# HuiGuanLab/Lite-MKD

Hardware: AMD Instinct MI355X
Metric: episodes/sec (5-way 5-shot, 8x224^2 frames) (higher is better)
Workload: dtype f32

## Files before the change

lite-mkd_amd/csrc/conv.hip:

```cpp
#include "gemm_core.h"
#include <atomic>
#include <mutex>

struct ConvGemmArgs {
  const float* src;
  const float* wpk;
  float* out;
  float* stat_partial;
  int N, Hs, Ws, Cs;
  int Hr, Wr, rows_per_class, tiles_per_class;
  int sh;
  int Ho, Wo, Co, omul;
  int Kp, cps, nclass;
  int n_rt, n_ct, xcd_mode;
  int taps_pm1;
  int grid_step;
  int grid_total;
  int same;
  int halo;
  int accum;
  const float* ep_stats;
  const float* ep_res;
  int ep_relu;
  const float* pre_stats;
// ... 130 lines not shown
    }
    if (ok) {
      s_src[r] = ((n * a.Hs + aa * a.sh) * a.Ws + bb * a.sh) * a.Cs;
      s_hw[r] = ((aa * a.sh) << 16) | (bb * a.sh);
      s_out[r] = ((n * a.Ho + aa * a.omul + ph) * a.Wo + bb * a.omul + pw) * a.Co;
    } else {
      s_src[r] = 0;
      s_hw[r] = -1;
      s_out[r] = -1;
    }
  }
  __syncthreads();
  LA la;
  LB lb;
  la.init(a.src, a.Hs, a.Ws, a.Cs, s_src, s_hw);
  lb.init(a.wpk, a.Kp, n0, a.Co, a.Kp);

  f32x16 acc[Cfg::TM][Cfg::TN];
  const int nk = a.ntap[cls] * a.cps;
  {
    constexpr int SA = LA::LDS_FLOATS, SB = LB::LDS_FLOATS;
    float* As0 = smem;
    float* Bs0 = smem + 2 * SA;
    const int lane = tid & 63, wave = tid >> 6;
    const int wm = wave / Cfg::WN, wn = wave % Cfg::WN;
    const int h = lane >> 5;
    const int a_row = wm * (Cfg::TM * 32) + (lane & 31);
    const int b_row = wn * (Cfg::TN * 32) + (lane & 31);
#pragma unroll
    for (int i = 0; i < Cfg::TM; ++i)
#pragma unroll
      for (int j = 0; j < Cfg::TN; ++j)
#pragma unroll
        for (int e = 0; e < 16; ++e) acc[i][j][e] = 0.f;
    const Tap* taps = a.taps[cls];
    const int ntap_c = a.ntap[cls];
    auto issue = [&](int t) {
      const int cc = t / ntap_c, tp = t - cc * ntap_c;
      const Tap tap = taps[tp];
      if (PRE && tp == 0) la.load_pre(a.pre_stats, cc * LMKD_BK);
      la.load(tap.dh, tap.dw, cc * LMKD_BK);
      lb.load(tap.kofs + cc * LMKD_BK);
    };
    if (nk > 0) {
      issue(0);
      la.store(As0);
      lb.store(Bs0);
      __syncthreads();
      for (int t = 0; t + 1 < nk; ++t) {
        const int cur = t & 1;
        issue(t + 1);
        if (BF16) mfma_kstep_bf16<Cfg, LA, LB>(As0 + cur * SA, Bs0 + cur * SB, a_row, b_row, h, acc);
        else mfma_kstep<Cfg, LA, LB>(As0 + cur * SA, Bs0 + cur * SB, a_row, b_row, h, acc);
        __builtin_amdgcn_sched_barrier(0);
        la.store(As0 + (cur ^ 1) * SA);
        lb.store(Bs0 + (cur ^ 1) * SB);
        __syncthreads();
      }
      const int last = (nk - 1) & 1;
      if (BF16) mfma_kstep_bf16<Cfg, LA, LB>(As0 + last * SA, Bs0 + last * SB, a_row, b_row, h, acc);
      else mfma_kstep<Cfg, LA, LB>(As0 + last * SA, Bs0 + last * SB, a_row, b_row, h, acc);
    }
  }

  const int lane = tid & 63, wave = tid >> 6;
  const int wm = wave / Cfg::WN, wn = wave % Cfg::WN;
  const int cl0 = wn * (Cfg::TN * 32) + (lane & 31);
  if (STATS == 0 && a.accum) {
    float prev[Cfg::TM][Cfg::TN][16];
#pragma unroll
    for (int i = 0; i < Cfg::TM; ++i)
#pragma unroll
      for (int e = 0; e < 16; ++e) {
        const int ob = s_out[wm * (Cfg::TM * 32) + i * 32 + acc_row(e, lane)];
#pragma unroll
        for (int j = 0; j < Cfg::TN; ++j) {
          const int col = n0 + cl0 + j * 32;
          prev[i][j][e] = (ob >= 0 && col < a.Co) ? a.out[(long)ob + col] : 0.f;
        }
      }
#pragma unroll
    for (int i = 0; i < Cfg::TM; ++i)
#pragma unroll
      for (int j = 0; j < Cfg::TN; ++j)
#pragma unroll
        for (int e = 0; e < 16; ++e) acc[i][j][e] = acc[i][j][e] + prev[i][j][e];
  }
  float s1[Cfg::TN], s2[Cfg::TN];
#pragma unroll
  for (int j = 0; j < Cfg::TN; ++j) s1[j] = s2[j] = 0.f;
  float esc[Cfg::TN], esh[Cfg::TN];
  if (STATS == 2) {
#pragma unroll
    for (int j = 0; j < Cfg::TN; ++j) {
      const int col = n0 + cl0 + j * 32;
      esc[j] = col < a.Co ? a.ep_stats[2 * a.Co + col] : 0.f;
      esh[j] = col < a.Co ? a.ep_stats[3 * a.Co + col] : 0.f;
    }
  }
#pragma unroll
  for (int i = 0; i < Cfg::TM; ++i) {
#pragma unroll
    for (int e = 0; e < 16; ++e) {
      const int rl = wm * (Cfg::TM * 32) + i * 32 + acc_row(e, lane);
      const int ob = s_out[rl];
#pragma unroll
      for (int j = 0; j < Cfg::TN; ++j) {
        const int col = n0 + cl0 + j * 32;
        float v = acc[i][j][e];
        if (ob >= 0 && col < a.Co) {
          float* o = a.out + (long)ob + col;
          if (STATS == 2) {
            v = fmaf(v, esc[j], esh[j]);
            if (a.ep_res) v += a.ep_res[(long)ob + col];
            if (a.ep_relu) v = fmaxf(v, 0.f);
            *o = v;
          } else {
            *o = (STATS == 1 && a.accum) ? v + *o : v;
          }
        }
        if (STATS == 1) { s1[j] += v; s2[j] = fmaf(v, v, s2[j]); }
      }
    }
    __builtin_amdgcn_sched_barrier(0);
  }
  if (STATS == 1) {
#pragma unroll
    for (int j = 0; j < Cfg::TN; ++j) {
      const float t1 = s1[j] + __shfl_xor(s1[j], 32, 64);
      const float t2 = s2[j] + __shfl_xor(s2[j], 32, 64);
      if (lane < 32) {
        s_red[(wm * Cfg::BN + cl0 + j * 32) * 2 + 0] = t1;
        s_red[(wm * Cfg::BN + cl0 + j * 32) * 2 + 1] = t2;
      }
    }
  }
  if (STATS == 1) {
    __syncthreads();
    if (tid < Cfg::BN && n0 + tid < a.Co) {
      float s1 = 0.f, s2 = 0.f;
#pragma unroll
      for (int w = 0; w < Cfg::WM; ++w) {
        s1 += s_red[(w * Cfg::BN + tid) * 2 + 0];
        s2 += s_red[(w * Cfg::BN + tid) * 2 + 1];
      }
      float* p = a.stat_partial + ((long)rt * a.Co + n0 + tid) * 2;
      p[0] = s1;
      p[1] = s2;
    }
  }
}

#include "conv_x3.h"
#include "h2.h"
#include "conv_patch.h"
#include "conv_patch16.h"
#include "conv_stem.h"

struct WgradArgs {
  const float* dy;
  const float* x;
  float* slab;
  int N, Hs, Ws, Cs, Ho, Wo, Co;
  int stride, pad, KH, KW, KWp;
  int Kp, Mpix, steps_total, steps_per_split;
  int n_mt, n_jt, splits, xcd_mode;
  const float* pre_stats;
  int seg_pix0, seg_splits0, sps1;
  FastDiv div_hw, div_w;
  const unsigned* h2_xw;
  const unsigned* h2_dyw;
};

struct WinSlab { int kfirst, kend, nk, seg; };
__device__ __forceinline__ WinSlab win_slab(int z, int Mpix, int sps0, int seg_pix0, int seg_splits0, int sps1) {
  WinSlab w;
  int sps;
  if (z < seg_splits0) { w.kfirst = z * sps0 * LMKD_BK; w.kend = seg_pix0; w.seg = 0; sps = sps0; }
  else { w.kfirst = seg_pix0 + (z - seg_splits0) * sps1 * LMKD_BK; w.kend = Mpix; w.seg = 1; sps = sps1; }
  const int left = (w.kend - w.kfirst + LMKD_BK - 1) / LMKD_BK;
  w.nk = left < sps ? (left < 0 ? 0 : left) : sps;
  return w;
}

template <int ROWS, bool SMALLC, int THREADS = LMKD_THREADS, bool PRE = false>
struct LoaderWgradGather {
  static constexpr bool ROWK = false;
  static constexpr int LD = ROWS;
  static constexpr int LDS_FLOATS = LMKD_BK * LD;
  static constexpr int CPR = ROWS / 4;
  static constexpr int KPP = THREADS / CPR;
  static constexpr int NI = LMKD_BK / KPP;
  const float* x;
  FastDiv div_hw, div_w;
  int Mpix, HoWo, Wo, Hs, Ws, Cs, stride;
  float4 reg[NI];
  int dh, dw, coff, r4;
  bool tap_ok;
  float4 psc, psh;
  unsigned inb;
  __device__ __forceinline__ void init(const WgradArgs& a, int j0) {
    inb = 0u;
    x = a.x; div_hw = a.div_hw; div_w = a.div_w;
    Mpix = a.Mpix; HoWo = a.Ho * a.Wo; Wo = a.Wo; Hs = a.Hs; Ws = a.Ws; Cs = a.Cs; stride = a.stride;
    const int tid = threadIdx.x;
    r4 = (tid % CPR) * 4;
    const int col = j0 + r4;
    if (SMALLC) {
      const int kh = col >> 5, kw = (col & 31) >> 2;
      dh = kh - a.pad; dw = kw - a.pad; coff = 0;
      tap_ok = kh < a.KH && kw < a.KW && col < a.Kp;
    } else {
      const int tap = col / a.Cs;
      coff = col - tap * a.Cs;
      const int kh = tap / a.KWp, kw = tap - kh * a.KWp;
      dh = kh - a.pad; dw = kw - a.pad;
      tap_ok = col < a.Kp && kw < a.KW;
    }
    if (PRE && tap_ok) {
      psc = *reinterpret_cast<const float4*>(a.pre_stats + 2 * a.Cs + coff);
      psh = *reinterpret_cast<const float4*>(a.pre_stats + 3 * a.Cs + coff);
    }
  }
  __device__ __forceinline__ void load(int koff) {
    const int tid = threadIdx.x;
#pragma unroll
    for (int i = 0; i < NI; ++i) {
      const int p = koff + tid / CPR + KPP * i;
      float4 v = make_float4(0.f, 0.f, 0.f, 0.f);
      if (tap_ok && p < Mpix) {
        const int n = fdiv(p, div_hw);
        const int rem = p - n * HoWo;
        const int oh = fdiv(rem, div_w);
        const int ow = rem - oh * Wo;
        const int h = oh * stride + dh, w = ow * stride + dw;
        if ((unsigned)h < (unsigned)Hs && (unsigned)w < (unsigned)Ws) {
          v = *reinterpret_cast<const float4*>(x + ((long)(n * Hs + h) * Ws + w) * Cs + coff);
          if (PRE) inb |= 1u << i;
        } else if (PRE) inb &= ~(1u << i);
      } else if (PRE) inb &= ~(1u << i);
      reg[i] = v;
    }
  }
  __device__ __forceinline__ void store(float* S) const {
    const int tid = threadIdx.x;
#pragma unroll
    for (int i = 0; i < NI; ++i) {
      int k = tid / CPR + KPP * i;
      float4 v = reg[i];
      if (PRE && ((inb >> i) & 1u)) {
        v.x = fmaxf(fmaf(v.x, psc.x, psh.x), 0.f); v.y = fmaxf(fmaf(v.y, psc.y, psh.y), 0.f);
        v.z = fmaxf(fmaf(v.z, psc.z, psh.z), 0.f); v.w = fmaxf(fmaf(v.w, psc.w, psh.w), 0.f);
      }
      *reinterpret_cast<float4*>(S + k * LD + r4) = v;
    }
  }
};

template <class Cfg, bool SMALLC, bool BF16, bool PRE = false>
__global__ __launch_bounds__(Cfg::THREADS) void conv_wgrad_kernel(WgradArgs a) {
  using LA = LoaderMMajorDense<Cfg::BM, Cfg::THREADS>;
  using LB = LoaderWgradGather<Cfg::BN, SMALLC, Cfg::THREADS, PRE>;
  __shared__ __attribute__((aligned(16))) float smem[2 * (LA::LDS_FLOATS + LB::LDS_FLOATS)];
  int z, tz;
  const int tiles_per_z = a.n_mt * a.n_jt;
  if (a.xcd_mode) {
    const int xj = blockIdx.x >> 3;
    z = (blockIdx.x & 7) + 8 * (xj / tiles_per_z);
    if (z >= a.splits) return;
    tz = xj - (xj / tiles_per_z) * tiles_per_z;
  } else {
    z = blockIdx.x / tiles_per_z;
    tz = blockIdx.x - z * tiles_per_z;
  }
  const int m0 = (tz % a.n_mt) * Cfg::BM, j0 = (tz / a.n_mt) * Cfg::BN;
  LA la;
  LB lb;
  la.init(a.dy, a.Co, m0, a.Co, a.Mpix);
  lb.init(a, j0);
  const int s0 = z * a.steps_per_split;
  int nk = a.steps_total - s0;
  if (nk > a.steps_per_split) nk = a.steps_per_split;
  f32x16 acc[Cfg::TM][Cfg::TN];
  auto koff = [s0](int t) { return (s0 + t) * LMKD_BK; };
  gemm_mainloop<Cfg, LA, LB, decltype(koff), decltype(koff), BF16, PRE>(la, lb, nk, koff, koff, smem, acc);

  const int lane = threadIdx.x & 63, wave = threadIdx.x >> 6;
  const int wm = wave / Cfg::WN, wn = wave % Cfg::WN;
  float* C = a.slab + (long)z * a.Co * a.Kp;
#pragma unroll
  for (int j = 0; j < Cfg::TN; ++j) {
    const int col = j0 + wn * (Cfg::TN * 32) + j * 32 + (lane & 31);
    if (col >= a.Kp) continue;
#pragma unroll
    for (int i = 0; i < Cfg::TM; ++i)
#pragma unroll
      for (int e = 0; e < 16; ++e) {
        const int row = m0 + wm * (Cfg::TM * 32) + i * 32 + acc_row(e, lane);
        if (row < a.Co) C[(long)row * a.Kp + col] = acc[i][j][e];
      }
  }
}

__global__ void wgrad_reduce_kernel(const float* __restrict__ slab, float* __restrict__ dw, int splits, int Co, int Cin,
                                    int Cs, int KH, int KW, int KWp, int Kp, int accumulate) {
  const long total = (long)Co * KH * KW * Cin;
  const long zs = (long)Co * Kp;
  for (long idx = (long)blockIdx.x * blockDim.x + threadIdx.x; idx < total; idx += (long)gridDim.x * blockDim.x) {
    const int ci = idx % Cin;
    long r = idx / Cin;
    const int kw = r % KW; r /= KW;
    const int kh = r % KH;
    const int co = r / KH;
    const float* p = slab + (long)co * Kp + (long)(kh * KWp + kw) * Cs + ci;
    float s0 = 0.f, s1 = 0.f, s2 = 0.f, s3 = 0.f;
    int z = 0;
    for (; z + 8 <= splits; z += 8) {
      const float a0 = p[(z + 0) * zs], a1 = p[(z + 1) * zs], a2 = p[(z + 2) * zs], a3 = p[(z + 3) * zs];
      const float a4 = p[(z + 4) * zs], a5 = p[(z + 5) * zs], a6 = p[(z + 6) * zs], a7 = p[(z + 7) * zs];
      s0 += a0; s1 += a1; s2 += a2; s3 += a3; s0 += a4; s1 += a5; s2 += a6; s3 += a7;
    }
    for (; z < splits; ++z) s0 += p[z * zs];
    float* o = dw + (((long)co * Cin + ci) * KH + kh) * KW + kw;
    const float v = (s0 + s1) + (s2 + s3);
    *o = accumulate ? *o + v : v;
  }
}

__global__ __launch_bounds__(1024) void wgrad_reduce_stem_kernel(const float* __restrict__ slab, float* __restrict__ dw, int splits, int Co, int Cin,
                                                                 int Cs, int KH, int KW, int KWp, int Kp, int accumulate) {
  __shared__ float sm[4][256];
  const int k = threadIdx.x, q = threadIdx.y, co = blockIdx.x;
  const long zs = (long)Co * Kp;
  float s0 = 0.f, s1 = 0.f, s2 = 0.f, s3 = 0.f;
  if (k < Kp) {
    const float* p = slab + (long)co * Kp + k;
    int z = q;
    for (; z + 28 < splits; z += 32) {
      const float a0 = p[(z + 0) * zs], a1 = p[(z + 4) * zs], a2 = p[(z + 8) * zs], a3 = p[(z + 12) * zs];
      const float a4 = p[(z + 16) * zs], a5 = p[(z + 20) * zs], a6 = p[(z + 24) * zs], a7 = p[(z + 28) * zs];
      s0 += a0; s1 += a1; s2 += a2; s3 += a3; s0 += a4; s1 += a5; s2 += a6; s3 += a7;
    }
    for (; z < splits; z += 4) s0 += p[z * zs];
  }
  sm[q][k] = (s0 + s1) + (s2 + s3);
  __syncthreads();
  if (q == 0 && k < Kp) {
    const int ci = k % Cs, r = k / Cs;
    const int kw = r % KWp, kh = r / KWp;
    if (ci < Cin && kw < KW && kh < KH) {
      const float v = (sm[0][k] + sm[1][k]) + (sm[2][k] + sm[3][k]);
      float* o = dw + (((long)co * Cin + ci) * KH + kh) * KW + kw;
      *o = accumulate ? *o + v : v;
    }
  }
}
static void launch_wgrad_reduce(const float* slab, float* dw, int splits, int Co, int Cin, int Cs, int KH, int KW, int KWp, int Kp,
                                int accumulate, hipStream_t s) {
  const long total = (long)Co * KH * KW * Cin;
  int rg = cdiv(total, 256);
  if (rg > 4096) rg = 4096;
  hipLaunchKernelGGL(wgrad_reduce_kernel, dim3(rg), dim3(256), 0, s, slab, dw, splits, Co, Cin, Cs, KH, KW, KWp, Kp, accumulate);
}

#include "wgrad_x3.h"
#include "wgrad_win.h"
#include "wgrad_stem.h"

__global__ void pack_weights_kernel(const float* __restrict__ w, float* __restrict__ wp, int Co, int Cin, int Cs, int KH,
                                    int KW, int KWp, int mode) {
  if (mode == 0) {
    const long total = (long)Co * KH * KWp * Cs;
    for (long idx = (long)blockIdx.x * blockDim.x + threadIdx.x; idx < total; idx += (long)gridDim.x * blockDim.x) {
      const int ci = idx % Cs;
      long r = idx / Cs;
      const int kw = r % KWp; r /= KWp;
      const int kh = r % KH;
      const int co = r / KH;
      wp[idx] = (ci < Cin && kw < KW) ? w[(((long)co * Cin + ci) * KH + kh) * KW + kw] : 0.f;
    }
  } else {
    const long total = (long)Cin * KH * KW * Co;
    for (long idx = (long)blockIdx.x * blockDim.x + threadIdx.x; idx < total; idx += (long)gridDim.x * blockDim.x) {
      const int co = idx % Co;
      long r = idx / Co;
      const int kw = r % KW; r /= KW;
      const int kh = r % KH;
      const int ci = r / KH;
      wp[idx] = w[(((long)co * Cin + ci) * KH + kh) * KW + kw];
    }
  }
}

static inline int conv_out(int H, int K, int s, int p) { return (H + 2 * p - K) / s + 1; }
static inline int kw_padded(int Cs, int KW) { return Cs >= 32 ? KW : ((KW * Cs + 31) / 32) * 32 / Cs; }

extern "C" long lmkd_conv2d_packed_weight_elems(int Cout, int Cin, int Cs, int KH, int KW, int mode) {
  if (mode == 0) return (long)Cout * KH * kw_padded(Cs, KW) * Cs;
  return (long)Cin * KH * KW * Cout;
}

extern "C" int lmkd_conv2d_pack_weights(const float* w_oihw, float* wp, int Cout, int Cin, int Cs, int KH, int KW,
                                        int mode, void* stream) {
  LMKD_REQUIRE(w_oihw && wp, "lmkd_conv2d_pack_weights: null pointer");
  LMKD_REQUIRE(mode == 0 || mode == 1, "lmkd_conv2d_pack_weights: mode must be 0 (fwd) or 1 (dgrad)");
  LMKD_REQUIRE(Cs >= Cin && (Cs % 32 == 0 || Cs == 4), "lmkd_conv2d_pack_weights: Cs=%d must be 4 or a multiple of 32", Cs);
  const long total = lmkd_conv2d_packed_weight_elems(Cout, Cin, Cs, KH, KW, mode);
  int grid = cdiv(total, 256);
  if (grid > 4096) grid = 4096;
  hipLaunchKernelGGL(pack_weights_kernel, dim3(grid), dim3(256), 0, (hipStream_t)stream, w_oihw, wp, Cout, Cin, Cs, KH, KW,
                     kw_padded(Cs, KW), mode);
  LMKD_CHECK_LAUNCH("lmkd_conv2d_pack_weights");
  return LMKD_OK;
}

static int g_conv_mode = 2;
static std::atomic<long> g_h2_launches{0};
static std::atomic<long> g_h2_fallbacks{0};
extern "C" long lmkd_conv_h2_launches(void) { return g_h2_launches.load(); }
extern "C" long lmkd_conv_h2_fallbacks(void) { return g_h2_fallbacks.load(); }
extern "C" int lmkd_conv_set_compute_dtype(int mode) {
  LMKD_REQUIRE(mode >= 0 && mode <= 4, "lmkd_conv_set_compute_dtype: 0 fp32 MFMA, 1 bf16, 2 fp32 as 3xbf16 (6 products), 3 (9 products), 4 fp32 as 2xfp16 (3 products) over mode 2");
  g_conv_mode = mode;
  return LMKD_OK;
}
extern "C" int lmkd_conv_get_compute_dtype(void) { return g_conv_mode; }
static inline int conv_nprod(bool act16 = false, bool maxima = false) {
  if (act16) return 1;
  switch (g_conv_mode) {
    case 0: return 0;
    case 1: return 1;
    case 3: return 9;
    case 4: return maxima ? 3 : 6;
    default: return 6;
  }
}
static inline bool conv_planes() { return conv_nprod() != 0; }
static inline bool conv_h2() { return conv_nprod(false, true) == 3; }
static inline void note_fenced(const lmkd_amax_desc* am) { if (conv_h2() && am && (am->flags & LMKD_AMAX_FENCED)) ++g_h2_fallbacks; }
extern "C" long lmkd_conv2d_plane_elems(int ncols, int Kp) {
  const long n = (long)ncols * Kp;
  return conv_nprod() == 1 ? n : (conv_h2() ? 18 * n + 32 : 12 * n);
}
static int amax_impl(const float* x, long n, void* word, int slots, void* stream, bool zero = true) {
  LMKD_REQUIRE(x && word && n > 0, "lmkd_amax: bad arguments");
  if (zero && hipMemsetAsync(word, 0, slots ? LMKD_AMAX_SEG_WORDS * 4 : 4, (hipStream_t)stream) != hipSuccess) {
    lmkd_set_error("lmkd_amax: hipMemsetAsync failed");
    return LMKD_EHIP;
  }
  int grid = cdiv(n, 256 * 16);
  if (grid > 2048) grid = 2048;
  if (slots) hipLaunchKernelGGL(amax_kernel<true>, dim3(grid), dim3(256), 0, (hipStream_t)stream, x, n, (unsigned*)word);
  else hipLaunchKernelGGL(amax_kernel<false>, dim3(grid), dim3(256), 0, (hipStream_t)stream, x, n, (unsigned*)word);
  LMKD_CHECK_LAUNCH("amax_kernel");
  return LMKD_OK;
}
extern "C" int lmkd_amax(const float* x, long n, void* word, void* stream) { return amax_impl(x, n, word, 1, stream); }

extern "C" int lmkd_conv2d_split_weights(const float* wp, void* wf, int ncols, int Kp, void* stream) {
  LMKD_REQUIRE(wp && wf, "lmkd_conv2d_split_weights: null pointer");
  LMKD_REQUIRE(ncols > 0 && ncols % 32 == 0 && Kp > 0 && Kp % 32 == 0, "lmkd_conv2d_split_weights: ncols=%d and Kp=%d must be multiples of 32", ncols, Kp);
  LMKD_REQUIRE((long)ncols * Kp * 24 < 0xffffffe0L, "lmkd_conv2d_split_weights: weights exceed the 4 GiB buffer range");
  int grid = cdiv((long)ncols * Kp, 256);
  if (grid > 4096) grid = 4096;
  hipLaunchKernelGGL(split_weights_kernel, dim3(grid), dim3(256), 0, (hipStream_t)stream, wp, (unsigned short*)wf, ncols, Kp,
                     conv_nprod() == 1 ? 1 : 3);
  LMKD_CHECK_LAUNCH("split_weights_kernel");
  if (conv_nprod() != 1) {
    hipLaunchKernelGGL(split_weights16_kernel, dim3(grid), dim3(256), 0, (hipStream_t)stream, wp, (unsigned short*)wf + (long)ncols * Kp * 6, ncols, Kp);
    LMKD_CHECK_LAUNCH("split_weights16_kernel");
  }
  if (conv_h2()) {
    unsigned short* wh = (unsigned short*)wf + (long)ncols * Kp * 12;
    const int rc = amax_impl(wp, (long)ncols * Kp, wh + (long)ncols * Kp * 4, 0, stream);
    if (rc) return rc;
    hipLaunchKernelGGL(split_weights16_h2_kernel, dim3(grid), dim3(256), 0, (hipStream_t)stream, wp, wh, ncols, Kp);
    LMKD_CHECK_LAUNCH("split_weights16_h2_kernel");
    hipLaunchKernelGGL(split_weights_h2_32_kernel, dim3(grid), dim3(256), 0, (hipStream_t)stream, wp, wh, ncols, Kp);
    LMKD_CHECK_LAUNCH("split_weights_h2_32_kernel");
  }
  return LMKD_OK;
}

struct RepackEntry {
  const float* w;
  unsigned short* wf;
  int Co, Cin, Cs, KH, KW, KWp, mode, ncols, Kp;
};
#define LMKD_REPACK_MAX 40
struct RepackArgs {
  RepackEntry e[LMKD_REPACK_MAX];
  int npl;
};
__device__ __forceinline__ float repack_fetch(const RepackEntry& e, int col, int k) {
  if (e.mode == 0) {
    const int ci = k % e.Cs;
    const int r = k / e.Cs;
    const int kw = r % e.KWp, kh = r / e.KWp;
    return (ci < e.Cin && kw < e.KW) ? e.w[(((long)col * e.Cin + ci) * e.KH + kh) * e.KW + kw] : 0.f;
  }
  const int co = k % e.Co;
  const int r = k / e.Co;
  const int kw = r % e.KW, kh = r / e.KW;
  return e.w[(((long)co * e.Cin + col) * e.KH + kh) * e.KW + kw];
}
__global__ void repack_h2_kernel(RepackArgs a, int phase) {
  const RepackEntry& e = a.e[blockIdx.y];
  const long total = (long)e.ncols * e.Kp;
  unsigned short* wh = e.wf + total * 12;
  unsigned* word = reinterpret_cast<unsigned*>(wh + total * 4);
  if (phase == 0) {
    if (blockIdx.x == 0 && threadIdx.x == 0) *word = 0u;
    return;
  }
  if (phase == 1) {
    float m = 0.f;
    for (long idx = (long)blockIdx.x * blockDim.x + threadIdx.x; idx < total; idx += (long)gridDim.x * blockDim.x) {
      const int col = (int)(idx / e.Kp), k = (int)(idx - (long)col * e.Kp);
      m = fmaxf(m, fabsf(repack_fetch(e, col, k)));
    }
#pragma unroll
    for (int o = 32; o >= 1; o >>= 1) m = fmaxf(m, __shfl_xor(m, o, 64));
    if ((threadIdx.x & 63) == 0) atomicMax(word, __float_as_uint(m));
    return;
  }
  const float s = h2_scale(*word);
  const int G16 = e.Kp >> 5, G = e.Kp >> 4;
  unsigned short* wh32 = wh + total * 4 + 32;
  for (long idx = (long)blockIdx.x * blockDim.x + threadIdx.x; idx < total; idx += (long)gridDim.x * blockDim.x) {
    const int col = (int)(idx / e.Kp), k = (int)(idx - (long)col * e.Kp);
    const int lane16 = (col & 15) + 16 * patch16_kslot((k >> 3) & 3);
    const long q = ((((long)(col >> 4) * G16 + (k >> 5)) * 2) * 64 + lane16) * 8 + (k & 7);
    unsigned short p0, p1;
    h2_split1(repack_fetch(e, col, k) * s, p0, p1);
    wh[q] = p0; wh[q + 512] = p1;
    const long q2 = q + total * 2;
    wh[q2] = p0 ^ 0x8000u; wh[q2 + 512] = p1 ^ 0x8000u;
    const long o = ((((long)(col >> 5) * G + (k >> 4)) * 2) * 64 + (col & 31) + 32 * ((k >> 3) & 1)) * 8 + (k & 7);
    wh32[o] = p0; wh32[o + 512] = p1;
  }
}
__global__ void repack_multi_kernel(RepackArgs a) {
  const RepackEntry& e = a.e[blockIdx.y];
  const long total = (long)e.ncols * e.Kp;
  const int G = e.Kp >> 4, G16 = e.Kp >> 5;
  for (long idx = (long)blockIdx.x * blockDim.x + threadIdx.x; idx < total; idx += (long)gridDim.x * blockDim.x) {
    const int col = (int)(idx / e.Kp), k = (int)(idx - (long)col * e.Kp);
    const float x = repack_fetch(e, col, k);
    const int lane = (col & 31) + 32 * ((k >> 3) & 1);
    const long o = ((((long)(col >> 5) * G + (k >> 4)) * a.npl) * 64 + lane) * 8 + (k & 7);
    if (a.npl == 1) {
      union { __bf16 h; unsigned short u; } c;
      c.h = (__bf16)x;
      e.wf[o] = c.u;
      continue;
    }
    const unsigned b0 = __float_as_uint(x);
    const float r1 = x - __uint_as_float(b0 & 0xffff0000u);
    const unsigned b1 = __float_as_uint(r1);
    const float r2 = r1 - __uint_as_float(b1 & 0xffff0000u);
    const unsigned short p0 = (unsigned short)(b0 >> 16), p1 = (unsigned short)(b1 >> 16), p2 = (unsigned short)(__float_as_uint(r2) >> 16);
    const unsigned short n0 = p0 ^ 0x8000u, n1 = p1 ^ 0x8000u, n2 = p2 ^ 0x8000u;
    e.wf[o] = p0; e.wf[o + 512] = p1; e.wf[o + 1024] = p2;
    const long o2 = o + total * 3;
    e.wf[o2] = n0; e.wf[o2 + 512] = n1; e.wf[o2 + 1024] = n2;
    unsigned short* w16 = e.wf + total * 6;
    const int lane16 = (col & 15) + 16 * patch16_kslot((k >> 3) & 3);
    const long q = ((((long)(col >> 4) * G16 + (k >> 5)) * 3) * 64 + lane16) * 8 + (k & 7);
    w16[q] = p0; w16[q + 512] = p1; w16[q + 1024] = p2;
    const long q2 = q + total * 3;
    w16[q2] = n0; w16[q2 + 512] = n1; w16[q2 + 1024] = n2;
  }
}

extern "C" int lmkd_conv2d_repack_multi(const float* const* ws, void* const* wfs, const int* dims, int n, void* stream) {
  LMKD_REQUIRE(ws && wfs && dims && n > 0, "lmkd_conv2d_repack_multi: null pointer");
  LMKD_REQUIRE(conv_planes(), "lmkd_conv2d_repack_multi: fragment-order planes exist in the bf16-plane modes only");
  for (int i0 = 0; i0 < n; i0 += LMKD_REPACK_MAX) {
    RepackArgs a;
    memset(&a, 0, sizeof(a));
    a.npl = conv_nprod() == 1 ? 1 : 3;
    const int m = std::min(LMKD_REPACK_MAX, n - i0);
    long most = 0;
    for (int j = 0; j < m; ++j) {
      const int* d = dims + (long)(i0 + j) * 6;
      RepackEntry& e = a.e[j];
      e.w = ws[i0 + j]; e.wf = (unsigned short*)wfs[i0 + j];
      e.Co = d[0]; e.Cin = d[1]; e.Cs = d[2]; e.KH = d[3]; e.KW = d[4]; e.mode = d[5];
      LMKD_REQUIRE(e.w && e.wf && (e.mode == 0 || e.mode == 1), "lmkd_conv2d_repack_multi: bad entry %d", i0 + j);
      LMKD_REQUIRE(e.Cs >= e.Cin && (e.Cs % 32 == 0 || e.Cs == 4), "lmkd_conv2d_repack_multi: Cs=%d must be 4 or a multiple of 32", e.Cs);
      e.KWp = kw_padded(e.Cs, e.KW);
      e.ncols = e.mode == 0 ? e.Co : e.Cin;
      e.Kp = e.mode == 0 ? e.KH * e.KWp * e.Cs : e.KH * e.KW * e.Co;
      LMKD_REQUIRE(e.ncols % 32 == 0 && e.Kp % 32 == 0, "lmkd_conv2d_repack_multi: entry %d: ncols=%d and Kp=%d must be multiples of 32", i0 + j, e.ncols, e.Kp);
      most = std::max(most, (long)e.ncols * e.Kp);
    }
    int gx = cdiv(most, 256 * 4);
    if (gx > 512) gx = 512;
    hipLaunchKernelGGL(repack_multi_kernel, dim3(gx, m), dim3(256), 0, (hipStream_t)stream, a);
    LMKD_CHECK_LAUNCH("repack_multi_kernel");
    if (conv_h2()) {
      for (int phase = 0; phase < 3; ++phase) {
        hipLaunchKernelGGL(repack_h2_kernel, dim3(phase == 0 ? 1 : gx, m), dim3(256), 0, (hipStream_t)stream, a, phase);
        LMKD_CHECK_LAUNCH("repack_h2_kernel");
      }
    }
  }
  return LMKD_OK;
}

static int g_tile_override = 0;
extern "C" int lmkd_conv_set_tile(int id) {
  LMKD_REQUIRE(id >= 0 && id <= 14, "lmkd_conv_set_tile: id must be 0 (auto) .. 14");
  g_tile_override = id;
  return LMKD_OK;
}
static inline int cfg_bm(int id) { return (id == 7 || id == 10 || id == 13 || id == 14) ? 256 : ((id <= 2 || id >= 5) ? 128 : 64); }
static inline int cfg_bn(int id) { return (id == 1 || id == 4 || id == 5 || id == 8 || id == 10 || id == 12 || id == 13) ? 128 : 64; }
static inline int cfg_wg_per_cu(int id) { return id == 1 ? 2 : (id == 3 ? 4 : 3); }

static int pick_conv_cfg(long rows_per_class, int nclass, int ncols, bool same = false) {
  if (conv_planes()) {
    if (g_tile_override >= 7) {
      int id = g_tile_override;
      if (id == 10 && !same) id = 8;
      if (id == 11 && !same) id = 9;
      if (id == 12 && !same) id = 8;
      if ((id == 13 || id == 14) && (!same || conv_nprod() != 1)) id = id == 13 ? 10 : 7;
      if (id == 10 && !same) id = 8;
      if (ncols <= 64 && cfg_bn(id) == 128) id = id == 10 ? 7 : (id == 12 ? 11 : (id == 13 ? 14 : 9));
      return id;
    }
    if (same) {
      if (ncols <= 64) return 11;
      const long t128 = cdiv(rows_per_class, 128) * cdiv(ncols, 128);
      return (conv_nprod() != 1 && t128 >= 1024) ? 12 : 11;
    }
    if (ncols <= 64) return 9;
    return (long)nclass * cdiv(rows_per_class, 128) * cdiv(ncols, 128) >= 256 ? 8 : 9;
  }
  if (g_tile_override) {
    if (ncols <= 64 && cfg_bn(g_tile_override) == 128) return g_tile_override == 5 ? 6 : (cfg_bm(g_tile_override) == 128 ? 2 : 3);
    return g_tile_override;
  }
  int best = 0;
  double best_cost = 1e30;
  const int cand[4] = {5, 2, 4, 3};
  for (int c = 0; c < 4; ++c) {
    const int id = cand[c];
    if (ncols <= 64 && cfg_bn(id) == 128) continue;
    const long tiles = (long)nclass * cdiv(rows_per_class, cfg_bm(id)) * cdiv(ncols, cfg_bn(id));
    double cost = (double)cdiv(tiles, 256) * cfg_bm(id) * cfg_bn(id);
    cost *= (id == 5 ? 0.92 : (id == 3 ? 1.00 : 1.07));
    if (nclass == 4 && id != 3) cost *= 1.5;
    if (cost < best_cost) { best_cost = cost; best = id; }
  }
  return best;
}

static inline void lmkd_lds_attr_once(std::atomic<unsigned long long>& mask, const void* fn, int bytes) {
  int d = 0;
  if (hipGetDevice(&d) != hipSuccess) d = 0;
  const unsigned long long bit = 1ull << (d & 63);
  if (mask.load(std::memory_order_acquire) & bit) return;
  const hipError_t err = hipFuncSetAttribute(fn, hipFuncAttributeMaxDynamicSharedMemorySize, bytes);
// ... 528 lines not shown
}

extern "C" int lmkd_conv2d_bwd_data(const float* dy, const float* wd, float* dx, int N, int H, int W, int Cin, int Cout,
                                    int KH, int KW, int stride, int pad, int accumulate, void* stream) {
  LMKD_REQUIRE(dy && wd && dx, "lmkd_conv2d_bwd_data: null pointer");
  LMKD_REQUIRE(aligned16(dy) && aligned16(wd), "lmkd_conv2d_bwd_data: operands must be 16-byte aligned");
  ConvGemmArgs a;
  if (const int rc = bwd_data_args(a, dy, wd, dx, N, H, W, Cin, Cout, KH, KW, stride, pad, accumulate)) return rc;
  return launch_conv(a, plan_dgrad(a), (hipStream_t)stream);
}

extern "C" int lmkd_conv2d_bwd_data_bn_tiles_seg(int N, int H, int W, int Cin, int Cout, int KH, int KW, int stride, int pad, int seg_n0, int* tiles0) {
  if (stride != 1 || Cout % 32 != 0 || KH * KW > LMKD_MAX_TAPS) return 0;
  ConvGemmArgs a;
  if (bwd_data_args(a, nullptr, nullptr, nullptr, N, H, W, Cin, Cout, KH, KW, stride, pad, 0, seg_n0)) return 0;
  const ConvPlan p = plan_dgrad(a);
  if (!p.bnb_form) return 0;
  if (tiles0) *tiles0 = p.seg_t0;
  return p.tiles_per_class;
}
extern "C" int lmkd_conv2d_bwd_data_bn_tiles(int N, int H, int W, int Cin, int Cout, int KH, int KW, int stride, int pad) {
  return lmkd_conv2d_bwd_data_bn_tiles_seg(N, H, W, Cin, Cout, KH, KW, stride, pad, 0, nullptr);
}
extern "C" int lmkd_conv2d_bwd_data_seg(const float* dy, const float* wd, float* dx, const float* bn_x, const float* bn_stats, float* part, int N,
                                        int H, int W, int Cin, int Cout, int KH, int KW, int stride, int pad, int accumulate, int seg_n0, void* stream,
                                        const lmkd_amax_desc* amax) {
  LMKD_REQUIRE(dy && wd && dx, "lmkd_conv2d_bwd_data_seg: null pointer");
  LMKD_REQUIRE(aligned16(dy) && aligned16(wd), "lmkd_conv2d_bwd_data_seg: operands must be 16-byte aligned");
  LMKD_REQUIRE((bn_x != nullptr) == (bn_stats != nullptr) && (bn_x != nullptr) == (part != nullptr), "lmkd_conv2d_bwd_data_seg: bn_x, bn_stats and part go together");
  ConvGemmArgs a;
  if (const int rc = bwd_data_args(a, dy, wd, dx, N, H, W, Cin, Cout, KH, KW, stride, pad, accumulate, seg_n0, amax)) return rc;
  note_fenced(amax);
  if (bn_x) {
    LMKD_REQUIRE(!accumulate && aligned16(bn_x) && aligned16(bn_stats), "lmkd_conv2d_bwd_data_seg: the fused BatchNorm sums need a plain (non-accumulating) launch and aligned operands");
    a.bnb_x = bn_x; a.bnb_stats = bn_stats; a.stat_partial = part;
  }
  const ConvPlan p = plan_dgrad(a);
  LMKD_REQUIRE(!bn_x || p.bnb_form, "lmkd_conv2d_bwd_data_seg: this launch has no fused form (lmkd_conv2d_bwd_data_bn_tiles_seg returned 0)");
  return launch_conv(a, p, (hipStream_t)stream);
}
extern "C" int lmkd_conv2d_bwd_data_bn(const float* dy, const float* wd, float* dx, const float* bn_x, const float* bn_stats, float* part,
                                       int N, int H, int W, int Cin, int Cout, int KH, int KW, int stride, int pad, void* stream) {
  LMKD_REQUIRE(dy && wd && dx && bn_x && bn_stats && part, "lmkd_conv2d_bwd_data_bn: null pointer");
  LMKD_REQUIRE(aligned16(dy) && aligned16(wd) && aligned16(bn_x) && aligned16(bn_stats), "lmkd_conv2d_bwd_data_bn: operands must be 16-byte aligned");
  ConvGemmArgs a;
  if (const int rc = bwd_data_args(a, dy, wd, dx, N, H, W, Cin, Cout, KH, KW, stride, pad, 0)) return rc;
  a.bnb_x = bn_x; a.bnb_stats = bn_stats; a.stat_partial = part;
  const ConvPlan p = plan_dgrad(a);
  LMKD_REQUIRE(p.bnb_form, "lmkd_conv2d_bwd_data_bn: this launch has no fused form (lmkd_conv2d_bwd_data_bn_tiles returned 0)");
  return launch_conv(a, p, (hipStream_t)stream);
}

static int g_wgrad_planes = 1;
extern "C" int lmkd_conv_set_wgrad_planes(int on) { g_wgrad_planes = on ? 1 : 0; return LMKD_OK; }
static int g_wgrad_win16 = 1;
extern "C" int lmkd_conv_set_wgrad_win16(int on) { g_wgrad_win16 = on ? 1 : 0; return LMKD_OK; }
static int g_wgrad_window = 1;
extern "C" int lmkd_conv_set_wgrad_window(int on) { g_wgrad_window = on < 0 ? 0 : on; return LMKD_OK; }
static inline bool wgrad_win_eligible(int W, int Cs, int Cout, int KH, int KW, int stride, int pad) {
  return g_wgrad_window && g_wgrad_planes && conv_planes() && KH == 3 && KW == 3 && stride == 1 && pad == 1 &&
         Cs % 32 == 0 && 32 + 2 * (W + 1) <= 256;
}
static void wgrad_win_plan(int Mpix, int W, int Cs, int Cout, int* cob, int* splits, int* steps_per_split) {
  *cob = Cout >= 128 ? 4 : 2;
  const int tiles = cdiv(Cout, 32 * *cob) * (Cs / 32);
  const int steps = cdiv(Mpix, LMKD_BK);
  const int warm = cdiv(2 * (W + 1), LMKD_BK);
  const int resident = 256 * ((conv_nprod() >= 6 && *cob == 2) ? 2 : 8 / *cob);
  int sp = g_wgrad_window > 1 ? cdiv(g_wgrad_window, tiles)
                              : std::max((int)(((long)resident * steps + 19600L * 4 / *cob) / (39200L * 4 / *cob)), cdiv(128, tiles));
  const int cap = std::max(1, steps / (12 * warm));
  if (sp > cap) sp = cap;
  *steps_per_split = cdiv(steps, sp);
  *splits = cdiv(steps, *steps_per_split);
}

static void wgrad_plan(int Mpix, int Cout, int Kp, int* splits, int* steps_per_split, int* bm, int* bn, bool planes = false) {
  *bm = Cout <= 64 ? 64 : 128;
  *bn = (Kp % 128 == 0 && Kp >= 1024) ? 128 : 64;
  int per_cu = (*bm == 128 && *bn == 128) ? 2 : ((*bm == 64 && *bn == 64) ? 4 : 3);
  if (planes) {
    if (*bm == 64 && *bn == 128) *bn = 64;
    const int npl = conv_nprod() == 1 ? 1 : 3;
    const long lds = 1L * npl * LMKD_BK * ((*bm * 2 + 64) + (*bn * 2 + 64));
    per_cu = (int)(160 * 1024 / lds);
    if (per_cu > 4) per_cu = 4;
    if (per_cu < 1) per_cu = 1;
  }
  const int tiles = cdiv(Cout, *bm) * cdiv(Kp, *bn);
  const int steps = cdiv(Mpix, LMKD_BK);
  const int slots = 256 * per_cu;
  int best_sp = 1;
  double best_cost = 1e30;
  for (int r = 1; r <= 3; ++r) {
    int sp = (slots * r) / tiles;
    if (sp > steps / 4) sp = steps / 4;
    if (sp < 1) sp = 1;
    const int sps = cdiv(steps, sp);
    sp = cdiv(steps, sps);
    const double rounds = (double)cdiv((long)tiles * sp, slots);
    const double cost = rounds * sps + 1.0 * sp / 8.0;
    if (cost < best_cost) { best_cost = cost; best_sp = sp; }
  }
  if (planes && *bm == 64 && *bn == 64 && best_sp < cdiv(steps, 64)) best_sp = cdiv(steps, 64);
  *steps_per_split = cdiv(steps, best_sp);
  *splits = cdiv(steps, *steps_per_split);
}

static int g_wgrad_stem = 1;
extern "C" int lmkd_conv_set_wgrad_stem(int on) { g_wgrad_stem = on ? 1 : 0; return LMKD_OK; }
static int stem_wgrad_plan(int N, int H, int W, int Cs, int Cout, int KH, int KW, int stride, int pad, int* G) {
  if (!g_wgrad_stem || !g_wgrad_planes || conv_nprod(g_lmkd_act_bf16) < 6 || Cs != 4 || Cout != 64 || KH != 7 || KW != 7 || stride != 2 || pad != 3) return 0;
  const int Ho = conv_out(H, KH, stride, pad), Wo = conv_out(W, KW, stride, pad);
  if (Wo < 17 || Wo > 128 || W > 2 * Wo || Ho < 1) return 0;
  const int units = N * cdiv(Ho, 2);
  int g = std::max(1, 2048 / (2 * Wo));
  g = std::min(g, std::max(1, units / 256));
  *G = g;
  return cdiv(units, g);
}

enum class WgFam : unsigned char {
  Stem,
  Win16,
  Win,
  Planes,
  Tile,
};
struct WgradPlan {
  WgFam fam;
  bool pre, act16, smallc;
  int nprod;
  int bm, bn;
  int cob;
  int G;
  int splits, splits0, sps0, sps1, seg_pix0;
  int xcd;
  int grid;
  long need;
  long ws;
};

static long wgrad_workspace(int N, int H, int W, int Cs, int Cout, int KH, int KW, int stride, int pad) {
  const int Ho = conv_out(H, KH, stride, pad), Wo = conv_out(W, KW, stride, pad);
  const int Kp = KH * kw_padded(Cs, KW) * Cs;
  int G, splits, sps, bm, bn;
  if (const int slabs = stem_wgrad_plan(N, H, W, Cs, Cout, KH, KW, stride, pad, &G)) return (long)slabs * Cout * Kp * sizeof(float);
  wgrad_plan(N * Ho * Wo, Cout, Kp, &splits, &sps, &bm, &bn, conv_planes() && g_wgrad_planes);
  if (wgrad_win_eligible(W, Cs, Cout, KH, KW, stride, pad)) {
    int cob, wsplits, wsps;
    wgrad_win_plan(N * Ho * Wo, W, Cs, Cout, &cob, &wsplits, &wsps);
    splits = std::max(splits, wsplits);
  }
  return (long)splits * Cout * Kp * sizeof(float);
}

static WgradPlan plan_wgrad(int N, int H, int W, int Cs, int Cout, int KH, int KW, int stride, int pad, int seg_n0, bool pre, bool maxima) {
  WgradPlan p;
  memset(&p, 0, sizeof(p));
  const bool act16 = g_lmkd_act_bf16;
  const int Ho = conv_out(H, KH, stride, pad), Wo = conv_out(W, KW, stride, pad);
  const int Kp = KH * kw_padded(Cs, KW) * Cs, Mpix = N * Ho * Wo;
  p.pre = pre; p.act16 = act16; p.smallc = Cs == 4;
  p.ws = wgrad_workspace(N, H, W, Cs, Cout, KH, KW, stride, pad);
  if (seg_n0)
    p.ws = std::max(p.ws, wgrad_workspace(seg_n0, H, W, Cs, Cout, KH, KW, stride, pad) + wgrad_workspace(N - seg_n0, H, W, Cs, Cout, KH, KW, stride, pad));
  p.seg_pix0 = seg_n0 ? seg_n0 * Ho * Wo : Mpix;
  if (const int slabs = stem_wgrad_plan(N, H, W, Cs, Cout, KH, KW, stride, pad, &p.G)) {
    p.fam = WgFam::Stem;
    p.nprod = conv_nprod(false, maxima);
    p.splits = p.grid = slabs;
  } else if (wgrad_win_eligible(W, Cs, Cout, KH, KW, stride, pad)) {
    const bool w16 = g_wgrad_win16 && conv_nprod(act16) >= 6;
    p.fam = w16 ? WgFam::Win16 : WgFam::Win;
    p.nprod = w16 ? conv_nprod(false, maxima) : conv_nprod(act16);
    wgrad_win_plan(Mpix, W, Cs, Cout, &p.cob, &p.splits, &p.sps0);
    p.splits0 = p.splits;
    if (seg_n0) {
      int sp1, cob1;
      wgrad_win_plan(p.seg_pix0, W, Cs, Cout, &p.cob, &p.splits0, &p.sps0);
      wgrad_win_plan(Mpix - p.seg_pix0, W, Cs, Cout, &cob1, &sp1, &p.sps1);
      p.splits = p.splits0 + sp1;
    }
    p.grid = 8 * cdiv(p.splits, 8) * cdiv(Cout, 32 * p.cob) * (Cs / 32);
  } else {
    const bool planes = conv_planes() && g_wgrad_planes;
    p.fam = planes ? WgFam::Planes : WgFam::Tile;
    p.nprod = planes ? conv_nprod(act16, maxima && !p.smallc && !pre) : (conv_nprod() == 1 ? 1 : 0);
    wgrad_plan(Mpix, Cout, Kp, &p.splits, &p.sps0, &p.bm, &p.bn, planes);
    p.splits0 = p.splits;
    if (seg_n0) {
      int sp1, bm1, bn1;
      wgrad_plan(p.seg_pix0, Cout, Kp, &p.splits0, &p.sps0, &p.bm, &p.bn, planes);
      wgrad_plan(Mpix - p.seg_pix0, Cout, Kp, &sp1, &p.sps1, &bm1, &bn1, planes);
      p.splits = p.splits0 + sp1;
    }
    p.xcd = (g_xcd_mode != 0 && g_xcd_mode != 1 && p.splits >= 32) ? 1 : 0;
    p.grid = (p.xcd ? 8 * cdiv(p.splits, 8) : p.splits) * cdiv(Cout, p.bm) * cdiv(Kp, p.bn);
  }
  p.need = (long)p.splits * Cout * Kp * sizeof(float);
  return p;
}

template <int NPROD, int D, int RLC>
static void launch_stem_wgrad(const StemWgradArgs& w, dim3 grid, size_t lds, hipStream_t s) {
  lds_attr_once<stem_wgrad_kernel<NPROD, D, RLC>>(160 * 1024);
  hipLaunchKernelGGL((stem_wgrad_kernel<NPROD, D, RLC>), grid, dim3(512), lds, s, w);
}
template <int NPROD>
static void launch_stem_wgrad(const StemWgradArgs& w, dim3 grid, size_t lds, hipStream_t s) {
  const bool deep = cdiv(2 * w.Wo, 32) >= 6;
  if (deep && w.RL == 1856) launch_stem_wgrad<NPROD, 6, 1856>(w, grid, lds, s);
  else if (deep) launch_stem_wgrad<NPROD, 6, 0>(w, grid, lds, s);
  else launch_stem_wgrad<NPROD, 2, 0>(w, grid, lds, s);
}
template <int COB>
static void launch_wgrad_win(const WgradWinArgs& w, const WgradPlan& p, bool big, hipStream_t s) {
  const dim3 grid(p.grid);
  if (p.fam == WgFam::Win16) {
    constexpr int JW = COB == 2 ? 1 : 2;
    constexpr int NT = 64 * COB * (2 / JW);
    with_nprod<3, 6, 9>(p.nprod, [&](auto np) {
      if (big && p.pre) hipLaunchKernelGGL((conv_wgrad_win16_kernel<COB, np, 256, true, 9, JW>), grid, dim3(NT), 0, s, w);
      else if (big) hipLaunchKernelGGL((conv_wgrad_win16_kernel<COB, np, 256, false, 9, JW>), grid, dim3(NT), 0, s, w);
      else if (p.pre) hipLaunchKernelGGL((conv_wgrad_win16_kernel<COB, np, 128, true, 9, JW>), grid, dim3(NT), 0, s, w);
      else hipLaunchKernelGGL((conv_wgrad_win16_kernel<COB, np, 128, false, 9, JW>), grid, dim3(NT), 0, s, w);
    });
    return;
  }
  auto go = [&](auto np, auto a16, auto pre) {
    constexpr int NPROD = decltype(np)::value;
    constexpr bool A16 = decltype(a16)::value, PRE = decltype(pre)::value;
    constexpr int TPW = (COB == 2 && NPROD != 1) ? 5 : 9;
    constexpr int NT = 64 * COB * ((9 + TPW - 1) / TPW);
    if (big) hipLaunchKernelGGL((conv_wgrad_win_kernel<COB, NPROD, A16, 256, PRE, TPW>), grid, dim3(NT), 0, s, w);
    else hipLaunchKernelGGL((conv_wgrad_win_kernel<COB, NPROD, A16, 128, PRE, TPW>), grid, dim3(NT), 0, s, w);
  };
  using T = std::true_type;
  using F = std::false_type;
  if (p.act16) go(std::integral_constant<int, 1>{}, T{}, F{});
  else with_nprod<1, 6, 9>(p.nprod, [&](auto np) { if (p.pre) go(np, F{}, T{}); else go(np, F{}, F{}); });
}

template <class CFG>
static void launch_wgrad_planes(const WgradArgs& a, const WgradPlan& p, hipStream_t s) {
  const dim3 grid(p.grid), block(256);
  if (p.act16) {
    if (p.smallc) hipLaunchKernelGGL((conv_wgrad_x3_kernel<CFG, true, 1, false, true>), grid, block, 0, s, a);
    else hipLaunchKernelGGL((conv_wgrad_x3_kernel<CFG, false, 1, false, true>), grid, block, 0, s, a);
  } else if (p.smallc) {
    with_nprod<1, 6, 9>(p.nprod, [&](auto np) { hipLaunchKernelGGL((conv_wgrad_x3_kernel<CFG, true, np, false>), grid, block, 0, s, a); });
  } else if (p.pre) {
    with_nprod<1, 6, 9>(p.nprod, [&](auto np) { hipLaunchKernelGGL((conv_wgrad_x3_kernel<CFG, false, np, true>), grid, block, 0, s, a); });
  } else {
    with_nprod<1, 3, 6, 9>(p.nprod, [&](auto np) { hipLaunchKernelGGL((conv_wgrad_x3_kernel<CFG, false, np, false>), grid, block, 0, s, a); });
  }
}

template <class CFG, bool SM, int THR>
static void launch_wgrad_tile(const WgradArgs& a, const WgradPlan& p, hipStream_t s) {
  const dim3 grid(p.grid);
  if (p.nprod == 1) hipLaunchKernelGGL((conv_wgrad_kernel<CFG, SM, true>), grid, dim3(THR), 0, s, a);
  else if (!SM && p.pre) hipLaunchKernelGGL((conv_wgrad_kernel<CFG, false, false, true>), grid, dim3(THR), 0, s, a);
  else hipLaunchKernelGGL((conv_wgrad_kernel<CFG, SM, false>), grid, dim3(THR), 0, s, a);
}

static int conv2d_bwd_weight_impl(const float* x, const float* pre_stats, const float* dy, float* dw_oihw, float* workspace,
                                  long ws_bytes, int N, int H, int W, int Cs, int Cin, int Cout, int KH, int KW, int stride, int pad,
                                  void* stream, int accumulate = 0, int seg_n0 = 0, const lmkd_amax_desc* am = nullptr) {
  const unsigned* amax_x = am ? (const unsigned*)am->x_words : nullptr;
  const unsigned* amax_dy = am ? (const unsigned*)am->dy_words : nullptr;
  note_fenced(am);
  LMKD_REQUIRE(x && dy && dw_oihw && workspace, "lmkd_conv2d_bwd_weight: null pointer");
  if (seg_n0 <= 0 || seg_n0 >= N) seg_n0 = 0;
  LMKD_REQUIRE(aligned16(x) && aligned16(dy) && aligned16(workspace), "lmkd_conv2d_bwd_weight: operands must be 16-byte aligned");
  LMKD_REQUIRE(Cs % 32 == 0 || Cs == 4, "lmkd_conv2d_bwd_weight: channel count %d must be 4 or a multiple of 32", Cs);
  LMKD_REQUIRE(Cout % 4 == 0, "lmkd_conv2d_bwd_weight: Cout %% 4 != 0");
  const bool smallc = Cs == 4;
  const WgradPlan p = plan_wgrad(N, H, W, Cs, Cout, KH, KW, stride, pad, seg_n0, pre_stats != nullptr, amax_x && amax_dy);
  LMKD_REQUIRE(!seg_n0 || p.fam != WgFam::Tile, "lmkd_conv2d_bwd_weight_seg: two frame segments exist in the bf16-plane modes");
  LMKD_REQUIRE(!pre_stats || (!smallc && (conv_nprod() != 1 || p.fam != WgFam::Tile) && !p.act16), "lmkd_conv2d_bwd_weight_pre: Cs %% 32 == 0, fp32 activations only");
  LMKD_REQUIRE(!p.act16 || (conv_nprod() == 1 && p.fam != WgFam::Tile), "bf16 activations need lmkd_conv_set_compute_dtype(1) and the plane weight-gradient kernel");
  const int Ho = conv_out(H, KH, stride, pad), Wo = conv_out(W, KW, stride, pad);
  const int KWp = kw_padded(Cs, KW), Kp = KH * KWp * Cs, Mpix = N * Ho * Wo;
  LMKD_REQUIRE((long)N * H * W * Cs < 2147483647L && (long)Mpix * Cout < 2147483647L, "lmkd_conv2d_bwd_weight: tensor too large");
  LMKD_REQUIRE(ws_bytes >= p.need, "lmkd_conv2d_bwd_weight: workspace too small");
  hipStream_t s = (hipStream_t)stream;
  if (p.fam == WgFam::Stem) {
    LMKD_REQUIRE((long)Mpix * 64 * 4 < 0xffffffe0L && (long)N * H * W * 16 < 0xffffffe0L, "lmkd_conv2d_bwd_weight: tensor too large for 32-bit byte offsets");
    StemWgradArgs w;
    memset(&w, 0, sizeof(w));
    w.dy = dy; w.x = x; w.slab = workspace;
    w.h2_xw = amax_x; w.h2_dyw = amax_dy;
    w.N = N; w.H = H; w.W = W; w.Ho = Ho; w.Wo = Wo;
    w.upi = cdiv(Ho, 2); w.units = N * w.upi; w.G = p.G; w.slabs = p.splits;
    w.RL = 16 * Wo + 64;
    const size_t lds = (size_t)2 * 10 * 3 * w.RL + 2 * 3 * STEM_WG_APLANE;
    with_nprod<3, 6, 9>(p.nprod, [&](auto np) { launch_stem_wgrad<np>(w, dim3(p.grid), lds, s); });
    LMKD_CHECK_LAUNCH("stem_wgrad_kernel");
    if (Kp <= 256) {
      hipLaunchKernelGGL(wgrad_reduce_stem_kernel, dim3(Cout), dim3(256, 4), 0, s, (const float*)workspace, dw_oihw, p.splits, Cout, Cin, Cs, KH, KW,
                         KWp, Kp, accumulate);
    } else {
      launch_wgrad_reduce((const float*)workspace, dw_oihw, p.splits, Cout, Cin, Cs, KH, KW, KWp, Kp, accumulate, s);
    }
    LMKD_CHECK_LAUNCH("wgrad_reduce_kernel");
    return LMKD_OK;
  }
  if (p.fam == WgFam::Win16 || p.fam == WgFam::Win) {
    LMKD_REQUIRE((long)Mpix * std::max(Cs, Cout) * 4 < 2147483647L, "lmkd_conv2d_bwd_weight: tensor too large for 32-bit byte offsets");
    WgradWinArgs w;
    memset(&w, 0, sizeof(w));
    w.dy = dy; w.x = x; w.slab = workspace; w.pre_stats = pre_stats;
    w.h2_xw = amax_x; w.h2_dyw = amax_dy;
    w.N = N; w.H = H; w.W = W; w.Cs = Cs; w.Co = Cout; w.Kp = Kp; w.Mpix = Mpix;
    w.steps_total = cdiv(Mpix, LMKD_BK);
    w.splits = p.splits; w.steps_per_split = p.sps0;
    w.seg_pix0 = p.seg_pix0; w.seg_splits0 = p.splits0; w.sps1 = p.sps1;
    w.n_ct = cdiv(Cout, 32 * p.cob); w.n_it = Cs / 32;
    w.div_hw = make_fastdiv(H * W); w.div_w = make_fastdiv(W);
    const bool big = 32 + 2 * (W + 1) > 128;
    if (p.cob == 4) launch_wgrad_win<4>(w, p, big, s);
    else launch_wgrad_win<2>(w, p, big, s);
    LMKD_CHECK_LAUNCH("conv_wgrad_win_kernel");
    launch_wgrad_reduce((const float*)workspace, dw_oihw, p.splits, Cout, Cin, Cs, KH, KW, KWp, Kp, accumulate, s);
    LMKD_CHECK_LAUNCH("wgrad_reduce_kernel");
    return LMKD_OK;
  }
  WgradArgs a;
  memset(&a, 0, sizeof(a));
  a.dy = dy; a.x = x; a.slab = workspace; a.pre_stats = pre_stats;
  a.h2_xw = amax_x; a.h2_dyw = amax_dy;
  a.N = N; a.Hs = H; a.Ws = W; a.Cs = Cs;
  a.Ho = Ho; a.Wo = Wo; a.Co = Cout;
  a.stride = stride; a.pad = pad; a.KH = KH; a.KW = KW; a.KWp = KWp;
  a.Kp = Kp; a.Mpix = Mpix;
  a.steps_per_split = p.sps0;
  a.seg_pix0 = p.seg_pix0; a.seg_splits0 = p.splits0; a.sps1 = p.sps1;
  a.steps_total = cdiv(Mpix, LMKD_BK);
  a.div_hw = make_fastdiv(Ho * Wo); a.div_w = make_fastdiv(Wo);
  a.n_mt = cdiv(Cout, p.bm); a.n_jt = cdiv(Kp, p.bn); a.splits = p.splits;
  a.xcd_mode = p.xcd;
  const int bm = p.bm, bn = p.bn;
  LMKD_REQUIRE(!smallc || (bm == 64 && bn == 64), "lmkd_conv2d_bwd_weight: padded-stem path expects Cout <= 64");
  if (p.fam == WgFam::Planes) {
    if (bm == 128 && bn == 128) launch_wgrad_planes<WgCfg<128, 128, 2, 2>>(a, p, s);
    else if (bm == 128) launch_wgrad_planes<WgCfg<128, 64, 2, 2>>(a, p, s);
    else launch_wgrad_planes<WgCfg<64, 64, 2, 2>>(a, p, s);
    LMKD_CHECK_LAUNCH("conv_wgrad_x3_kernel");
  } else {
    if (smallc) launch_wgrad_tile<TileCfg<64, 64, 2, 2>, true, LMKD_THREADS>(a, p, s);
    else if (bm == 64 && bn == 64) launch_wgrad_tile<TileCfg<64, 64, 2, 2>, false, LMKD_THREADS>(a, p, s);
    else if (bm == 128 && bn == 64) launch_wgrad_tile<TileCfg<128, 64, 2, 2>, false, LMKD_THREADS>(a, p, s);
    else if (bm == 64 && bn == 128) launch_wgrad_tile<TileCfg<64, 128, 2, 2>, false, LMKD_THREADS>(a, p, s);
    else launch_wgrad_tile<TileCfg<128, 128, 2, 4>, false, 512>(a, p, s);
    LMKD_CHECK_LAUNCH("conv_wgrad_kernel");
  }
  launch_wgrad_reduce((const float*)workspace, dw_oihw, p.splits, Cout, Cin, Cs, KH, KW, KWp, Kp, accumulate, s);
  LMKD_CHECK_LAUNCH("wgrad_reduce_kernel");
  return LMKD_OK;
}

extern "C" long lmkd_conv2d_bwd_weight_workspace_seg(int N, int H, int W, int Cs, int Cout, int KH, int KW, int stride, int pad, int seg_n0) {
  if (seg_n0 <= 0 || seg_n0 >= N) seg_n0 = 0;
  return plan_wgrad(N, H, W, Cs, Cout, KH, KW, stride, pad, seg_n0, false, false).ws;
}
extern "C" long lmkd_conv2d_bwd_weight_workspace(int N, int H, int W, int Cs, int Cout, int KH, int KW, int stride, int pad) {
  return lmkd_conv2d_bwd_weight_workspace_seg(N, H, W, Cs, Cout, KH, KW, stride, pad, 0);
}

extern "C" int lmkd_conv2d_bwd_weight(const float* x, const float* dy, float* dw_oihw, float* workspace, long ws_bytes,
                                      int N, int H, int W, int Cs, int Cin, int Cout, int KH, int KW, int stride, int pad,
                                      void* stream) {
  return conv2d_bwd_weight_impl(x, nullptr, dy, dw_oihw, workspace, ws_bytes, N, H, W, Cs, Cin, Cout, KH, KW, stride, pad, stream);
}

extern "C" int lmkd_conv2d_bwd_weight_pre(const float* x_raw, const float* pre_stats, const float* dy, float* dw_oihw,
                                          float* workspace, long ws_bytes, int N, int H, int W, int Cs, int Cin, int Cout, int KH,
                                          int KW, int stride, int pad, void* stream) {
  LMKD_REQUIRE(pre_stats, "lmkd_conv2d_bwd_weight_pre: BatchNorm table of the input missing");
  return conv2d_bwd_weight_impl(x_raw, pre_stats, dy, dw_oihw, workspace, ws_bytes, N, H, W, Cs, Cin, Cout, KH, KW, stride, pad, stream);
}

extern "C" int lmkd_conv2d_bwd_weight_acc(const float* x, const float* pre_stats, const float* dy, float* dw_oihw, float* workspace,
                                          long ws_bytes, int N, int H, int W, int Cs, int Cin, int Cout, int KH, int KW, int stride,
                                          int pad, void* stream) {
  return conv2d_bwd_weight_impl(x, pre_stats, dy, dw_oihw, workspace, ws_bytes, N, H, W, Cs, Cin, Cout, KH, KW, stride, pad, stream, 1);
}


extern "C" int lmkd_conv2d_bwd_weight_seg(const float* x, const float* pre_stats, const float* dy, float* dw_oihw, float* workspace, long ws_bytes,
                                          int N, int H, int W, int Cs, int Cin, int Cout, int KH, int KW, int stride, int pad, int accumulate,
                                          int seg_n0, void* stream, const lmkd_amax_desc* amax) {
  return conv2d_bwd_weight_impl(x, pre_stats, dy, dw_oihw, workspace, ws_bytes, N, H, W, Cs, Cin, Cout, KH, KW, stride, pad, stream, accumulate, seg_n0, amax);
}

extern "C" int lmkd_conv2d_plan(int kind, int N, int H, int W, int Cs, int Cin, int Cout, int KH, int KW, int stride, int pad,
                                int* info) {
  LMKD_REQUIRE(info && kind >= 0 && kind <= 2, "lmkd_conv2d_plan: kind must be 0 (forward), 1 (data gradient) or 2 (weight gradient)");
  LMKD_REQUIRE(N > 0 && H > 0 && W > 0 && Cout > 0 && KH > 0 && KW > 0 && stride > 0, "lmkd_conv2d_plan: bad shape");
  if (kind == 2) {
    const WgradPlan p = plan_wgrad(N, H, W, Cs, Cout, KH, KW, stride, pad, 0, false, false);
    info[1] = p.xcd; info[2] = p.splits; info[3] = p.grid;
    switch (p.fam) {
      case WgFam::Stem: info[0] = 14; info[4] = 2; break;
      case WgFam::Win16:
      case WgFam::Win: info[0] = p.cob == 4 ? 5 : 6; info[1] = 1; info[4] = 1; break;
      default: info[0] = (p.bm == 128 && p.bn == 128) ? 1 : (p.bm == 128 ? 2 : (p.bn == 128 ? 4 : 3)); info[4] = 0; break;
    }
    return LMKD_OK;
  }
  ConvGemmArgs a;
  if (kind == 0) fwd_geometry(a, N, H, W, Cs, Cout, KH, KW, stride, pad, 0);
  else dgrad_geometry(a, N, H, W, Cin, Cout, KH, KW, stride, pad, 0);
  const ConvPlan p = kind == 0 ? plan_fwd(a, KH, KW, pad) : plan_dgrad(a);
  info[0] = p.tile; info[1] = p.xcd; info[2] = p.nclass; info[3] = p.grid;
  info[4] = p.fam == ConvFam::Stem ? 2 : (p.fam == ConvFam::Patch || p.fam == ConvFam::Patch16 || p.fam == ConvFam::Patch1p ? 1 : 0);
  return LMKD_OK;
}
```

lite-mkd_amd/csrc/norm_pool.hip:

```cpp
#include "common.h"
#include <vector>
#include <cmath>
#include <algorithm>

#define NP_THREADS 256
static int g_ew_wg_per_cu = 4;
extern "C" int lmkd_set_elementwise_wg_per_cu(int n) {
  LMKD_REQUIRE(n >= 1 && n <= 8, "lmkd_set_elementwise_wg_per_cu: %d outside 1..8 (the BatchNorm partial buffers hold 2048 rows)", n);
  g_ew_wg_per_cu = n;
  return LMKD_OK;
}
static inline int ew_grid(long n_items) {
  long g = (n_items + NP_THREADS - 1) / NP_THREADS;
  if (g > 256 * g_ew_wg_per_cu) g = 256 * g_ew_wg_per_cu;
  if (g < 1) g = 1;
  return (int)g;
}

extern "C" long lmkd_amax_words(void) { return 2 * LMKD_AMAX_SEG_WORDS; }
static inline unsigned* amd_out(const lmkd_amax_desc* d) { return d ? (unsigned*)d->out_words : nullptr; }
static inline const unsigned* amd_ref(const lmkd_amax_desc* d) { return (d && d->out_words) ? (const unsigned*)d->ref_words : nullptr; }

#define LMKD_FENCE_MAX 128
struct FenceArgs { const unsigned* w[LMKD_FENCE_MAX]; unsigned* r[LMKD_FENCE_MAX]; };
__global__ void h2_fence_eval_kernel(FenceArgs a, int* __restrict__ flags) {
  const unsigned* w = a.w[blockIdx.x];
  unsigned* r = a.r[blockIdx.x];
  int f = 0;
  for (int seg = 0; seg < 2; ++seg) {
    const unsigned* slot = w + seg * LMKD_AMAX_SEG_WORDS + (threadIdx.x & (LMKD_AMAX_SLOTS - 1)) * LMKD_AMAX_STRIDE;
    unsigned long long ns = slot[1], q = *reinterpret_cast<const unsigned long long*>(slot + 2);
#pragma unroll
    for (int o = 32; o >= 1; o >>= 1) {
      ns += (unsigned long long)__shfl_xor((long long)ns, o, 64);
      q += (unsigned long long)__shfl_xor((long long)q, o, 64);
    }
    const unsigned cb = amax_read(w, seg), rb = amax_read(r, seg);
    const float cur = __uint_as_float(cb), ref = __uint_as_float(rb);
    if (ref > 0.f && cur >= 0.25f * ref && ns > 0 && 4 * ns > q) f |= 1 << seg;
    if (threadIdx.x == 0) r[seg * LMKD_AMAX_SEG_WORDS] = cb;
  }
  if (threadIdx.x == 0) flags[blockIdx.x] = f;
}
extern "C" int lmkd_h2_fence_eval(const void* const* words, void* const* refs, int n, int* flags, void* stream) {
  LMKD_REQUIRE(words && refs && flags && n > 0, "lmkd_h2_fence_eval: bad arguments");
  for (int i0 = 0; i0 < n; i0 += LMKD_FENCE_MAX) {
    FenceArgs a;
    const int m = std::min(LMKD_FENCE_MAX, n - i0);
    for (int j = 0; j < m; ++j) {
      LMKD_REQUIRE(words[i0 + j] && refs[i0 + j], "lmkd_h2_fence_eval: null entry %d", i0 + j);
      a.w[j] = (const unsigned*)words[i0 + j];
      a.r[j] = (unsigned*)refs[i0 + j];
    }
    for (int j = m; j < LMKD_FENCE_MAX; ++j) { a.w[j] = nullptr; a.r[j] = nullptr; }
    hipLaunchKernelGGL(h2_fence_eval_kernel, dim3(m), dim3(64), 0, (hipStream_t)stream, a, flags + i0);
    LMKD_CHECK_LAUNCH("h2_fence_eval_kernel");
  }
  return LMKD_OK;
}

__global__ void nchw3_to_nhwc4_kernel(const float* __restrict__ x, float4* __restrict__ y, long npix_total, long hw, unsigned* __restrict__ amax) {
  float am = 0.f;
  for (long p = (long)blockIdx.x * blockDim.x + threadIdx.x; p < npix_total; p += (long)gridDim.x * blockDim.x) {
    const long n = p / hw, r = p - n * hw;
    const float* b = x + n * 3 * hw + r;
    const float4 v = make_float4(b[0], b[hw], b[2 * hw], 0.f);
    y[p] = v;
    am = amax4(am, v);
  }
  if (amax) amax_commit(amax, am);
}

extern "C" int lmkd_nchw3_to_nhwc4(const float* x, float* y, int N, int H, int W, void* stream, void* amax_words) {
  unsigned* amax = (unsigned*)amax_words;
  LMKD_REQUIRE(x && y && N > 0 && H > 0 && W > 0, "lmkd_nchw3_to_nhwc4: bad arguments");
  LMKD_REQUIRE(aligned16(y), "lmkd_nchw3_to_nhwc4: output must be 16-byte aligned");
  const long hw = (long)H * W, total = hw * N;
  hipLaunchKernelGGL(nchw3_to_nhwc4_kernel, dim3(ew_grid(total)), dim3(NP_THREADS), 0, (hipStream_t)stream, x, (float4*)y, total, hw, amax);
  LMKD_CHECK_LAUNCH("lmkd_nchw3_to_nhwc4");
  return LMKD_OK;
}

__global__ void frames_u8_to_nhwc4_kernel(const unsigned char* __restrict__ src, float4* __restrict__ dst, const int* __restrict__ crop_y,
                                          const int* __restrict__ crop_x, const int* __restrict__ flip, long total, int Hs, int Ws,
                                          int H, int W, int frames_per_video) {
  for (long p = (long)blockIdx.x * blockDim.x + threadIdx.x; p < total; p += (long)gridDim.x * blockDim.x) {
    const int w = (int)(p % W);
    long r = p / W;
    const int h = (int)(r % H);
    const int f = (int)(r / H);
    const int v = f / frames_per_video;
    const int sx = crop_x[v] + (flip[v] ? (W - 1 - w) : w);
    const int sy = crop_y[v] + h;
    const unsigned char* s = src + (((long)f * Hs + sy) * Ws + sx) * 3;
    dst[p] = make_float4((float)s[0] / 255.f, (float)s[1] / 255.f, (float)s[2] / 255.f, 0.f);
  }
}

extern "C" int lmkd_frames_u8_to_nhwc4(const unsigned char* src, float* dst, const int* crop_y, const int* crop_x, const int* flip,
                                       int F, int Hs, int Ws, int H, int W, int frames_per_video, void* stream) {
  LMKD_REQUIRE(src && dst && crop_y && crop_x && flip && F > 0 && H > 0 && W > 0 && H <= Hs && W <= Ws && frames_per_video > 0,
               "lmkd_frames_u8_to_nhwc4: bad arguments");
  const long total = (long)F * H * W;
  hipLaunchKernelGGL(frames_u8_to_nhwc4_kernel, dim3(ew_grid(total)), dim3(NP_THREADS), 0, (hipStream_t)stream, src, (float4*)dst, crop_y,
                     crop_x, flip, total, Hs, Ws, H, W, frames_per_video);
  LMKD_CHECK_LAUNCH("frames_u8_to_nhwc4_kernel");
  return LMKD_OK;
}

#define LMKD_PIL_PRECISION_BITS 22

extern "C" int lmkd_resize_plan(int in_size, int out_size, int* bounds , int* coeffs ) {
  LMKD_REQUIRE(in_size > 0 && out_size > 0, "lmkd_resize_plan: sizes must be positive");
  const double scale = (double)in_size / out_size;
  const double filterscale = scale < 1.0 ? 1.0 : scale;
  const double support = 1.0 * filterscale;
  const int ksize = (int)ceil(support) * 2 + 1;
  if (!bounds || !coeffs) return ksize;
  const double ss = 1.0 / filterscale;
  std::vector<double> w(ksize);
  for (int xx = 0; xx < out_size; ++xx) {
    const double center = (xx + 0.5) * scale;
    int xmin = (int)(center - support + 0.5);
    if (xmin < 0) xmin = 0;
    int xmax = (int)(center + support + 0.5);
    if (xmax > in_size) xmax = in_size;
    xmax -= xmin;
    double ww = 0.0;
    for (int x = 0; x < ksize; ++x) w[x] = 0.0;
    for (int x = 0; x < xmax; ++x) {
      double a = (x + xmin - center + 0.5) * ss;
      if (a < 0.0) a = -a;
      w[x] = a < 1.0 ? 1.0 - a : 0.0;
      ww += w[x];
    }
    for (int x = 0; x < xmax; ++x)
      if (ww != 0.0) w[x] /= ww;
    for (int x = 0; x < ksize; ++x)
      coeffs[xx * ksize + x] = w[x] < 0 ? (int)(-0.5 + w[x] * (1 << LMKD_PIL_PRECISION_BITS)) : (int)(0.5 + w[x] * (1 << LMKD_PIL_PRECISION_BITS));
    bounds[xx * 2] = xmin;
    bounds[xx * 2 + 1] = xmax;
  }
  return ksize;
}

__global__ void resize_pass_u8_kernel(const unsigned char* __restrict__ src, unsigned char* __restrict__ dst, const int* __restrict__ bounds,
                                      const int* __restrict__ coeffs, int ksize, long total, int n_in, int n_out, long inner) {
  for (long p = (long)blockIdx.x * blockDim.x + threadIdx.x; p < total; p += (long)gridDim.x * blockDim.x) {
    const long i = p % inner;
    const long r = p / inner;
    const int xx = (int)(r % n_out);
    const long o = r / n_out;
    const int x0 = bounds[xx * 2], n = bounds[xx * 2 + 1];
    const unsigned char* s = src + (o * n_in + x0) * inner + i;
    const int* k = coeffs + (long)xx * ksize;
    int acc = 1 << (LMKD_PIL_PRECISION_BITS - 1);
    for (int x = 0; x < n; ++x) acc += (int)s[(long)x * inner] * k[x];
    acc >>= LMKD_PIL_PRECISION_BITS;
    dst[p] = (unsigned char)(acc < 0 ? 0 : (acc > 255 ? 255 : acc));
  }
}

extern "C" int lmkd_resize_pass_u8(const unsigned char* src, unsigned char* dst, const int* bounds_dev, const int* coeffs_dev, int ksize,
                                   long outer, int n_in, int n_out, long inner, void* stream) {
  LMKD_REQUIRE(src && dst && bounds_dev && coeffs_dev && ksize > 0 && outer > 0 && n_in > 0 && n_out > 0 && inner > 0,
               "lmkd_resize_pass_u8: bad arguments");
  const long total = outer * n_out * inner;
  hipLaunchKernelGGL(resize_pass_u8_kernel, dim3(ew_grid(total)), dim3(NP_THREADS), 0, (hipStream_t)stream, src, dst, bounds_dev, coeffs_dev,
                     ksize, total, n_in, n_out, inner);
  LMKD_CHECK_LAUNCH("resize_pass_u8_kernel");
  return LMKD_OK;
}

__global__ void frames_resize_crop_nhwc4_kernel(const unsigned char* __restrict__ src, float4* __restrict__ dst,
                                                const int* __restrict__ bh, const int* __restrict__ kh, int ksh,
                                                const int* __restrict__ bv, const int* __restrict__ kv, int ksv,
                                                const int* __restrict__ crop_y, const int* __restrict__ crop_x, const int* __restrict__ flip,
                                                int Hs, int Ws, int H, int W, int frames_per_video) {
  const int f = blockIdx.y;
  const int p = blockIdx.x * blockDim.x + threadIdx.x;
  if (p >= H * W) return;
  const int h = p / W, w = p - h * W;
  const int v = f / frames_per_video;
  const int sx = crop_x[v] + (flip[v] ? (W - 1 - w) : w);
  const int sy = crop_y[v] + h;
  const int x0 = bh[sx * 2], nx = bh[sx * 2 + 1];
  const int y0 = bv[sy * 2], ny = bv[sy * 2 + 1];
  const int* ch = kh + (long)sx * ksh;
  const int* cv = kv + (long)sy * ksv;
  int a0 = 1 << (LMKD_PIL_PRECISION_BITS - 1), a1 = a0, a2 = a0;
  for (int yy = 0; yy < ny; ++yy) {
    const unsigned char* row = src + (((long)f * Hs + y0 + yy) * Ws + x0) * 3;
    int t0 = 1 << (LMKD_PIL_PRECISION_BITS - 1), t1 = t0, t2 = t0;
    for (int xx = 0; xx < nx; ++xx) {
      const int k = ch[xx];
      t0 += (int)row[xx * 3 + 0] * k;
      t1 += (int)row[xx * 3 + 1] * k;
      t2 += (int)row[xx * 3 + 2] * k;
    }
    t0 >>= LMKD_PIL_PRECISION_BITS; t1 >>= LMKD_PIL_PRECISION_BITS; t2 >>= LMKD_PIL_PRECISION_BITS;
    t0 = t0 < 0 ? 0 : (t0 > 255 ? 255 : t0); t1 = t1 < 0 ? 0 : (t1 > 255 ? 255 : t1); t2 = t2 < 0 ? 0 : (t2 > 255 ? 255 : t2);
    const int k = cv[yy];
    a0 += t0 * k; a1 += t1 * k; a2 += t2 * k;
  }
  a0 >>= LMKD_PIL_PRECISION_BITS; a1 >>= LMKD_PIL_PRECISION_BITS; a2 >>= LMKD_PIL_PRECISION_BITS;
  a0 = a0 < 0 ? 0 : (a0 > 255 ? 255 : a0); a1 = a1 < 0 ? 0 : (a1 > 255 ? 255 : a1); a2 = a2 < 0 ? 0 : (a2 > 255 ? 255 : a2);
  dst[(long)f * H * W + p] = make_float4((float)a0 / 255.f, (float)a1 / 255.f, (float)a2 / 255.f, 0.f);
}

extern "C" int lmkd_frames_resize_crop_nhwc4(const unsigned char* src, float* dst, const int* bounds_h, const int* coeffs_h, int ksize_h,
                                             const int* bounds_v, const int* coeffs_v, int ksize_v, const int* crop_y, const int* crop_x,
                                             const int* flip, int F, int Hs, int Ws, int Hr, int Wr, int H, int W, int frames_per_video,
                                             void* stream) {
  LMKD_REQUIRE(src && dst && bounds_h && coeffs_h && bounds_v && coeffs_v && crop_y && crop_x && flip && ksize_h > 0 && ksize_v > 0 && F > 0 &&
               F <= 65535 && Hs > 0 && Ws > 0 && H > 0 && W > 0 && H <= Hr && W <= Wr && frames_per_video > 0, "lmkd_frames_resize_crop_nhwc4: bad arguments");
  hipLaunchKernelGGL(frames_resize_crop_nhwc4_kernel, dim3(cdiv(H * W, NP_THREADS), F), dim3(NP_THREADS), 0, (hipStream_t)stream, src,
                     (float4*)dst, bounds_h, coeffs_h, ksize_h, bounds_v, coeffs_v, ksize_v, crop_y, crop_x, flip, Hs, Ws, H, W, frames_per_video);
  LMKD_CHECK_LAUNCH("frames_resize_crop_nhwc4_kernel");
  return LMKD_OK;
}

#define CS_COLS 32
#define CS_LANES 8
#define CS_MAX_SLICES 64
#define LMKD_TICKET_WORDS 512
extern "C" long lmkd_ticket_words(void) { return LMKD_TICKET_WORDS; }

static inline int cs_slices(int T) { return T <= 64 ? 1 : std::min(CS_MAX_SLICES, cdiv(T, 64)); }

template <bool PROD = false>
__device__ __forceinline__ bool colsum_ticket(const float* __restrict__ in, int T, int CV, double* __restrict__ scratch,
                                              unsigned* __restrict__ tickets, double (*sm)[CS_COLS], double* tot, int* s_last,
                                              const float* __restrict__ in2 = nullptr, int S_ = 0) {
  const int tx = threadIdx.x, ty = threadIdx.y;
  const int col = blockIdx.x * CS_COLS + tx;
  const bool act = col < CV;
  const int S = S_ > 0 ? S_ : gridDim.y;
  if ((int)blockIdx.y >= S) return false;
  const int per = (T + S - 1) / S;
  const int t0 = blockIdx.y * per;
  const int t1 = t0 + per < T ? t0 + per : T;
  double s0 = 0.0, s1 = 0.0, s2 = 0.0, s3 = 0.0;
  if (act) {
    int t = t0 + ty;
    auto at = [&](int r) -> double {
      const long i = (long)r * CV + col;
      return PROD ? (double)(in[i] * in2[i]) : (double)in[i];
    };
    for (; t + 3 * CS_LANES < t1; t += 4 * CS_LANES) {
      s0 += at(t);
      s1 += at(t + CS_LANES);
      s2 += at(t + 2 * CS_LANES);
      s3 += at(t + 3 * CS_LANES);
    }
    for (; t < t1; t += CS_LANES) s0 += at(t);
  }
  sm[ty][tx] = (s0 + s1) + (s2 + s3);
  __syncthreads();
  double v = 0.0;
  if (ty == 0)
    for (int q = 0; q < CS_LANES; ++q) v += sm[q][tx];
  if (S == 1) {
    if (ty == 0) tot[tx] = v;
    __syncthreads();
    return true;
  }
  if (ty == 0 && act) __hip_atomic_store(&scratch[(long)blockIdx.y * CV + col], v, __ATOMIC_RELAXED, __HIP_MEMORY_SCOPE_AGENT);
  asm volatile("s_waitcnt vmcnt(0)" ::: "memory");
  __syncthreads();
  if (tx == 0 && ty == 0) *s_last = atomicAdd(&tickets[blockIdx.x], 1u) == (unsigned)(S - 1);
  __syncthreads();
  if (!*s_last) return false;
  asm volatile("" ::: "memory");
  {
    double a0 = 0.0, a1 = 0.0;
    if (act) {
      const double* sp = scratch + col;
      int q = ty;
      for (; q + CS_LANES < S; q += 2 * CS_LANES) {
        a0 += __hip_atomic_load(&sp[(long)q * CV], __ATOMIC_RELAXED, __HIP_MEMORY_SCOPE_AGENT);
        a1 += __hip_atomic_load(&sp[(long)(q + CS_LANES) * CV], __ATOMIC_RELAXED, __HIP_MEMORY_SCOPE_AGENT);
      }
      if (q < S) a0 += __hip_atomic_load(&sp[(long)q * CV], __ATOMIC_RELAXED, __HIP_MEMORY_SCOPE_AGENT);
    }
    sm[ty][tx] = a0 + a1;
  }
  __syncthreads();
  if (ty == 0) {
    double a = 0.0;
    for (int q = 0; q < CS_LANES; ++q) a += sm[q][tx];
    tot[tx] = a;
  }
  if (tx == 0 && ty == 0) tickets[blockIdx.x] = 0u;
  __syncthreads();
  return true;
}

__global__ void bn_finalize_kernel(const float* __restrict__ part, int T, int C, double count, const float* __restrict__ gamma,
                                   const float* __restrict__ beta, float* __restrict__ running_mean, float* __restrict__ running_var,
                                   float momentum, float eps, float* __restrict__ stats, double* __restrict__ scratch,
                                   unsigned* __restrict__ tickets, int T0 = 0, double count1 = 0.0, int S0 = 0, int S1 = 0,
                                   const unsigned* __restrict__ c_words = nullptr, unsigned* __restrict__ bound_words = nullptr,
                                   const unsigned* __restrict__ ref_words = nullptr) {
  __shared__ double sm[CS_LANES][CS_COLS];
  __shared__ double tot[CS_COLS];
  __shared__ int s_last;
  int S = 0;
  if (gridDim.z > 1) {
    if (blockIdx.z) {
      part += (long)T0 * 2 * C; T -= T0; count = count1; stats += 5 * C; scratch += (long)CS_MAX_SLICES * 2 * C; tickets += LMKD_TICKET_WORDS / 2; S = S1;
      if (c_words) { c_words += LMKD_AMAX_SEG_WORDS; bound_words += LMKD_AMAX_SEG_WORDS; }
      if (ref_words) ref_words += LMKD_AMAX_SEG_WORDS;
    } else { T = T0; S = S0; }
  }
  if (!colsum_ticket(part, T, 2 * C, scratch, tickets, sm, tot, &s_last, nullptr, S)) return;
  const int c = blockIdx.x * (CS_COLS / 2) + threadIdx.x;
  if (threadIdx.y != 0 || threadIdx.x >= CS_COLS / 2 || c >= C) return;
  const double s1 = tot[2 * threadIdx.x], s2 = tot[2 * threadIdx.x + 1];
  const double mean = s1 / count;
  double var = s2 / count - mean * mean;
  if (var < 0.0) var = 0.0;
  const float invstd = (float)(1.0 / sqrt(var + (double)eps));
  const float g = gamma ? gamma[c] : 1.f, b = beta ? beta[c] : 0.f;
  stats[c] = (float)mean;
  stats[C + c] = invstd;
  stats[2 * C + c] = g * invstd;
  stats[3 * C + c] = b - (float)mean * g * invstd;
  const double unb = count > 1.0 ? var * count / (count - 1.0) : var;
  stats[4 * C + c] = (float)unb;
  if (c_words) {
    unsigned gm = 0u;
    for (int s = 0; s < LMKD_AMAX_SLOTS; ++s) {
      const unsigned u = c_words[s * LMKD_AMAX_STRIDE];
      gm = u > gm ? u : gm;
    }
    if (gm) {
      const float bnd = fabsf(g * invstd) * __uint_as_float(gm) + fabsf(b - (float)mean * g * invstd);
      unsigned* slot = bound_words + (c & (LMKD_AMAX_SLOTS - 1)) * LMKD_AMAX_STRIDE;
      atomicMax(slot, __float_as_uint(bnd));
      if (ref_words) {
        unsigned rm = 0u;
        for (int q = 0; q < LMKD_AMAX_SLOTS; ++q) {
          const unsigned u = ref_words[q * LMKD_AMAX_STRIDE];
          rm = u > rm ? u : rm;
        }
        const AmaxRef rf = amax_ref(rm);
        const float typ = sqrtf(g * g + b * b);
        if (rf.thr > 0.f && typ > 0.f) {
          if (typ < rf.thr) atomicAdd(slot + 1, 1u);
          atomicAdd(reinterpret_cast<unsigned long long*>(slot + 2), (unsigned long long)(fminf(typ * rf.inv_thr, 1024.f) + 0.5f));
        }
      }
    }
  }
  if (running_mean) {
    running_mean[c] = (1.f - momentum) * running_mean[c] + momentum * (float)mean;
    running_var[c] = (1.f - momentum) * running_var[c] + momentum * (float)unb;
  }
}

__global__ void bn_running_update_kernel(float* __restrict__ running_mean, float* __restrict__ running_var,
                                         const float* __restrict__ stats, int C, float momentum) {
  const int c = blockIdx.x * blockDim.x + threadIdx.x;
  if (c >= C) return;
  running_mean[c] = (1.f - momentum) * running_mean[c] + momentum * stats[c];
  running_var[c] = (1.f - momentum) * running_var[c] + momentum * stats[4 * C + c];
}
extern "C" int lmkd_bn_running_update(float* running_mean, float* running_var, const float* stats, int C, float momentum,
                                      void* stream) {
  LMKD_REQUIRE(running_mean && running_var && stats && C > 0, "lmkd_bn_running_update: bad arguments");
  hipLaunchKernelGGL(bn_running_update_kernel, dim3(cdiv(C, 64)), dim3(64), 0, (hipStream_t)stream, running_mean, running_var,
                     stats, C, momentum);
  LMKD_CHECK_LAUNCH("bn_running_update_kernel");
  return LMKD_OK;
}

#define BN_MULTI_MAX 64
struct BnMultiArgs {
  float* rm[BN_MULTI_MAX];
  float* rv[BN_MULTI_MAX];
  const float* st0[BN_MULTI_MAX];
  const float* st1[BN_MULTI_MAX];
  long long* nbt[BN_MULTI_MAX];
  int C[BN_MULTI_MAX];
};
__global__ void bn_running_update_multi_kernel(BnMultiArgs a, float momentum) {
  const int b = blockIdx.x;
  const int C = a.C[b];
  if (threadIdx.x == 0 && a.nbt[b]) *a.nbt[b] += a.st1[b] ? 2 : 1;
  for (int c = threadIdx.x; c < C; c += blockDim.x) {
    float m = a.rm[b][c], v = a.rv[b][c];
    m = (1.f - momentum) * m + momentum * a.st0[b][c];
    v = (1.f - momentum) * v + momentum * a.st0[b][4 * C + c];
    if (a.st1[b]) {
      m = (1.f - momentum) * m + momentum * a.st1[b][c];
      v = (1.f - momentum) * v + momentum * a.st1[b][4 * C + c];
    }
    a.rm[b][c] = m;
    a.rv[b][c] = v;
  }
}
extern "C" int lmkd_bn_running_update_multi_nbt(float* const* running_mean, float* const* running_var, const float* const* stats_first,
                                                const float* const* stats_second, long long* const* num_batches_tracked, const int* C, int n,
                                                float momentum, void* stream);
extern "C" int lmkd_bn_running_update_multi(float* const* running_mean, float* const* running_var, const float* const* stats_first,
                                            const float* const* stats_second, const int* C, int n, float momentum, void* stream) {
  return lmkd_bn_running_update_multi_nbt(running_mean, running_var, stats_first, stats_second, nullptr, C, n, momentum, stream);
}
extern "C" int lmkd_bn_running_update_multi_nbt(float* const* running_mean, float* const* running_var, const float* const* stats_first,
                                                const float* const* stats_second, long long* const* num_batches_tracked, const int* C, int n,
                                                float momentum, void* stream) {
  LMKD_REQUIRE(running_mean && running_var && stats_first && stats_second && C && n > 0, "lmkd_bn_running_update_multi: bad arguments");
  for (int i0 = 0; i0 < n; i0 += BN_MULTI_MAX) {
    BnMultiArgs a;
    memset(&a, 0, sizeof(a));
    const int m = std::min(BN_MULTI_MAX, n - i0);
    for (int i = 0; i < m; ++i) {
      LMKD_REQUIRE(running_mean[i0 + i] && running_var[i0 + i] && stats_first[i0 + i] && C[i0 + i] > 0, "lmkd_bn_running_update_multi: null entry %d", i0 + i);
      a.rm[i] = running_mean[i0 + i]; a.rv[i] = running_var[i0 + i];
      a.st0[i] = stats_first[i0 + i]; a.st1[i] = stats_second[i0 + i];
      a.nbt[i] = num_batches_tracked ? num_batches_tracked[i0 + i] : nullptr;
      a.C[i] = C[i0 + i];
    }
    hipLaunchKernelGGL(bn_running_update_multi_kernel, dim3(m), dim3(256), 0, (hipStream_t)stream, a, momentum);
    LMKD_CHECK_LAUNCH("bn_running_update_multi_kernel");
  }
  return LMKD_OK;
}

__global__ void bn_eval_stats_kernel(int C, const float* __restrict__ gamma, const float* __restrict__ beta,
                                     const float* __restrict__ running_mean, const float* __restrict__ running_var, float eps,
                                     float* __restrict__ stats) {
  const int c = blockIdx.x * blockDim.x + threadIdx.x;
  if (c >= C) return;
  const float invstd = 1.f / sqrtf(running_var[c] + eps);
  const float g = gamma ? gamma[c] : 1.f, b = beta ? beta[c] : 0.f;
  stats[c] = running_mean[c];
  stats[C + c] = invstd;
  stats[2 * C + c] = g * invstd;
  stats[3 * C + c] = b - running_mean[c] * g * invstd;
  stats[4 * C + c] = running_var[c];
}

extern "C" int lmkd_bn_finalize(const float* partial, int T, int C, long count, const float* gamma, const float* beta,
                                float* running_mean, float* running_var, float momentum, float eps, float* stats,
                                double* scratch, unsigned* tickets, void* stream, const lmkd_amax_desc* amd) {
  const unsigned* bin = amd ? (const unsigned*)amd->x_words : nullptr;
  unsigned* bout = amd ? (unsigned*)amd->out_words : nullptr;
  if (!bin || !bout) { bin = nullptr; bout = nullptr; }
  LMKD_REQUIRE(partial && stats && scratch && tickets && T > 0 && C > 0 && count > 0, "lmkd_bn_finalize: bad arguments");
  LMKD_REQUIRE(cdiv(2 * C, CS_COLS) <= LMKD_TICKET_WORDS, "lmkd_bn_finalize: C=%d exceeds the ticket buffer", C);
  hipLaunchKernelGGL(bn_finalize_kernel, dim3(cdiv(2 * C, CS_COLS), cs_slices(T)), dim3(CS_COLS, CS_LANES), 0, (hipStream_t)stream, partial, T,
                     C, (double)count, gamma, beta, running_mean, running_var, momentum, eps, stats, scratch, tickets, 0, 0.0, 0, 0, bin, bout,
                     bout && amd ? (const unsigned*)amd->ref_words : nullptr);
  LMKD_CHECK_LAUNCH("bn_finalize_kernel");
  return LMKD_OK;
}

extern "C" int lmkd_bn_finalize_seg(const float* partial, int T, int T0, int C, long count0, long count1, const float* gamma, const float* beta,
                                    float eps, float* stats, double* scratch, unsigned* tickets, void* stream, const lmkd_amax_desc* amd) {
  const unsigned* bin = amd ? (const unsigned*)amd->x_words : nullptr;
  unsigned* bout = amd ? (unsigned*)amd->out_words : nullptr;
  if (!bin || !bout) { bin = nullptr; bout = nullptr; }
  LMKD_REQUIRE(partial && stats && scratch && tickets && T0 > 0 && T > T0 && C > 0 && count0 > 0 && count1 > 0, "lmkd_bn_finalize_seg: bad arguments");
  LMKD_REQUIRE(cdiv(2 * C, CS_COLS) <= LMKD_TICKET_WORDS / 2, "lmkd_bn_finalize_seg: C=%d exceeds the ticket buffer", C);
  const int S0 = cs_slices(T0), S1 = cs_slices(T - T0);
  hipLaunchKernelGGL(bn_finalize_kernel, dim3(cdiv(2 * C, CS_COLS), std::max(S0, S1), 2), dim3(CS_COLS, CS_LANES), 0, (hipStream_t)stream, partial, T,
                     C, (double)count0, gamma, beta, (float*)nullptr, (float*)nullptr, 0.f, eps, stats, scratch, tickets, T0, (double)count1, S0, S1, bin, bout,
                     bout && amd ? (const unsigned*)amd->ref_words : nullptr);
  LMKD_CHECK_LAUNCH("bn_finalize_kernel");
  return LMKD_OK;
}

extern "C" int lmkd_bn_eval_stats(int C, const float* gamma, const float* beta, const float* running_mean,
                                  const float* running_var, float eps, float* stats, void* stream) {
  LMKD_REQUIRE(running_mean && running_var && stats && C > 0, "lmkd_bn_eval_stats: bad arguments");
  hipLaunchKernelGGL(bn_eval_stats_kernel, dim3(cdiv(C, 64)), dim3(64), 0, (hipStream_t)stream, C, gamma, beta, running_mean,
                     running_var, eps, stats);
  LMKD_CHECK_LAUNCH("bn_eval_stats_kernel");
  return LMKD_OK;
}

template <typename T>
__global__ void bn_apply_kernel(const T* __restrict__ x, const float* __restrict__ stats, const T* __restrict__ res,
                                const float* __restrict__ rstats, T* __restrict__ y, long n4, int C, int relu, int res_mode,
                                unsigned* __restrict__ mask_bits, long n4_0, unsigned* __restrict__ amax, const unsigned* __restrict__ aref) {
  constexpr int U = ActU<T>::U;
  const int C4 = C >> 2;
  const long nu = n4 / U;
  AmaxStat am = {0.f, 0.f, 0u}, am1 = {0.f, 0.f, 0u};
  const AmaxRef rf0 = amax_ref(aref ? amax_read(aref, 0) : 0u), rf1 = amax_ref(aref ? amax_read(aref, 1) : 0u);
  for (long iu = (long)blockIdx.x * blockDim.x + threadIdx.x; iu < nu; iu += (long)gridDim.x * blockDim.x) {
    float4 v[U], r[U];
    ldv<T, U>(x, iu, v);
    if (res_mode) ldv<T, U>(res, iu, r);
    unsigned nibs = 0;
    const int so = iu * U >= n4_0 ? 5 * C : 0;
#pragma unroll
    for (int u = 0; u < U; ++u) {
      const long i = iu * U + u;
      const int c = (int)(i % C4) * 4 + so;
      const float4 sc = *reinterpret_cast<const float4*>(stats + 2 * C + c);
      const float4 sh = *reinterpret_cast<const float4*>(stats + 3 * C + c);
      float4& w = v[u];
      w.x = fmaf(w.x, sc.x, sh.x); w.y = fmaf(w.y, sc.y, sh.y); w.z = fmaf(w.z, sc.z, sh.z); w.w = fmaf(w.w, sc.w, sh.w);
      if (res_mode == 1) {
        w.x += r[u].x; w.y += r[u].y; w.z += r[u].z; w.w += r[u].w;
      } else if (res_mode == 2) {
        const float4 rs = *reinterpret_cast<const float4*>(rstats + 2 * C + c);
        const float4 rh = *reinterpret_cast<const float4*>(rstats + 3 * C + c);
        w.x += fmaf(r[u].x, rs.x, rh.x); w.y += fmaf(r[u].y, rs.y, rh.y); w.z += fmaf(r[u].z, rs.z, rh.z); w.w += fmaf(r[u].w, rs.w, rh.w);
      }
      if (relu) { w.x = fmaxf(w.x, 0.f); w.y = fmaxf(w.y, 0.f); w.z = fmaxf(w.z, 0.f); w.w = fmaxf(w.w, 0.f); }
      nibs |= ((w.x > 0.f ? 1u : 0u) | (w.y > 0.f ? 2u : 0u) | (w.z > 0.f ? 4u : 0u) | (w.w > 0.f ? 8u : 0u)) << (4 * u);
      if (so) amax_stat4(am1, w, rf1); else amax_stat4(am, w, rf0);
    }
    stv<T, U>(y, iu, v);
    if (mask_bits) {
      constexpr int LPW = 8 / U;
      unsigned wbits = nibs << (4 * U * (threadIdx.x & (LPW - 1)));
      wbits |= __shfl_xor(wbits, 1, 64);
      wbits |= __shfl_xor(wbits, 2, 64);
      if (LPW == 8) wbits |= __shfl_xor(wbits, 4, 64);
      if ((threadIdx.x & (LPW - 1)) == 0) mask_bits[iu / LPW] = wbits;
    }
  }
  if (amax) {
    amax_commit_stat(amax, am, aref != nullptr);
    if (n4_0 < n4) amax_commit_stat(amax + LMKD_AMAX_SEG_WORDS, am1, aref != nullptr);
  }
}

extern "C" int lmkd_bn_apply_seg(const float* x, const float* stats, const float* res, const float* rstats, float* y, long rows, long rows0,
                                 int C, int relu, int res_mode, unsigned* mask_bits, void* stream, const lmkd_amax_desc* amd);
extern "C" int lmkd_bn_apply(const float* x, const float* stats, const float* res, const float* rstats, float* y, long rows,
                             int C, int relu, int res_mode, unsigned* mask_bits, void* stream) {
  return lmkd_bn_apply_seg(x, stats, res, rstats, y, rows, rows, C, relu, res_mode, mask_bits, stream, nullptr);
}
extern "C" int lmkd_bn_apply_seg(const float* x, const float* stats, const float* res, const float* rstats, float* y, long rows, long rows0,
                                 int C, int relu, int res_mode, unsigned* mask_bits, void* stream, const lmkd_amax_desc* amd) {
  unsigned* amax = amd_out(amd);
  const unsigned* aref = amd_ref(amd);
  LMKD_REQUIRE(x && stats && y && rows > 0 && C > 0 && C % 4 == 0, "lmkd_bn_apply: bad arguments (C=%d)", C);
  if (rows0 <= 0 || rows0 > rows) rows0 = rows;
  LMKD_REQUIRE(res_mode == 0 || res, "lmkd_bn_apply: residual pointer missing");
  LMKD_REQUIRE(res_mode != 2 || rstats, "lmkd_bn_apply: residual stats missing");
  LMKD_REQUIRE(!mask_bits || C % 32 == 0, "lmkd_bn_apply: the ReLU bit mask needs C %% 32 == 0 (C=%d)", C);
  LMKD_REQUIRE(!g_lmkd_act_bf16 || C % 8 == 0, "lmkd_bn_apply: bf16 tensors need C %% 8 == 0 (C=%d)", C);
  const long n4 = rows * C / 4;
  if (g_lmkd_act_bf16)
    hipLaunchKernelGGL(bn_apply_kernel<lmkd_bf16_t>, dim3(ew_grid(n4)), dim3(NP_THREADS), 0, (hipStream_t)stream, (const lmkd_bf16_t*)x, stats,
                       (const lmkd_bf16_t*)res, rstats, (lmkd_bf16_t*)y, n4, C, relu, res_mode, mask_bits, rows0 * C / 4, amax, aref);
  else
    hipLaunchKernelGGL(bn_apply_kernel<float>, dim3(ew_grid(n4)), dim3(NP_THREADS), 0, (hipStream_t)stream, x, stats, res, rstats, y, n4, C,
                       relu, res_mode, mask_bits, rows0 * C / 4, amax, aref);
  LMKD_CHECK_LAUNCH("bn_apply_kernel");
  return LMKD_OK;
}

template <typename T>
__device__ __forceinline__ float4 bn_masked_grad(const float4 dy, const float4 xv, const T* yact, long i, const float* stats,
                                                 int C, int c, int mask_mode) {
  float4 g = dy;
  if (mask_mode == 3) {
    const unsigned nib = (reinterpret_cast<const unsigned*>(yact)[i >> 3] >> (4 * (int)(i & 7))) & 15u;
    g.x = (nib & 1u) ? g.x : 0.f; g.y = (nib & 2u) ? g.y : 0.f; g.z = (nib & 4u) ? g.z : 0.f; g.w = (nib & 8u) ? g.w : 0.f;
  } else if (mask_mode == 1) {
    const float4 yv = ld4<T>(yact, i);
    g.x = yv.x > 0.f ? g.x : 0.f; g.y = yv.y > 0.f ? g.y : 0.f; g.z = yv.z > 0.f ? g.z : 0.f; g.w = yv.w > 0.f ? g.w : 0.f;
  } else if (mask_mode == 2) {
    const float4 sc = *reinterpret_cast<const float4*>(stats + 2 * C + c);
    const float4 sh = *reinterpret_cast<const float4*>(stats + 3 * C + c);
    g.x = fmaf(xv.x, sc.x, sh.x) > 0.f ? g.x : 0.f; g.y = fmaf(xv.y, sc.y, sh.y) > 0.f ? g.y : 0.f;
    g.z = fmaf(xv.z, sc.z, sh.z) > 0.f ? g.z : 0.f; g.w = fmaf(xv.w, sc.w, sh.w) > 0.f ? g.w : 0.f;
  }
  return g;
}

struct BnSeg { long rows0; int nb1; };
template <typename T>
__global__ void bn_bwd_reduce_kernel(const T* __restrict__ dy, const T* __restrict__ x, const T* __restrict__ yact,
                                     const float* __restrict__ stats, float* __restrict__ partial, long rows, int C, int CC,
                                     int mask_mode, int nbv, BnSeg sg) {
  extern __shared__ float sm[];
  constexpr int U = ActU<T>::U;
  if (gridDim.z > 1) {
    if (blockIdx.z) {
      const long eo = sg.rows0 * C;
      dy += eo; x += eo;
      if (yact) yact = mask_mode == 3 ? reinterpret_cast<const T*>(reinterpret_cast<const unsigned*>(yact) + eo / 32) : yact + eo;
      stats += 5 * C; partial += (long)2048 * 2 * C; rows -= sg.rows0; nbv = sg.nb1;
    } else {
      rows = sg.rows0;
    }
  }
  const int C4 = C >> 2, CCV = CC / (4 * U);
  const int RL = NP_THREADS / CCV, RL1 = RL / U;
  const int cq = threadIdx.x % CCV, rl = threadIdx.x / CCV;
  const int bv = blockIdx.x * U + rl / RL1, vl = rl % RL1;
  const int c0 = blockIdx.y * CC;
  const int c = c0 + cq * 4 * U;
  float4 s1[U], s2[U], mean[U], istd[U];
#pragma unroll
  for (int u = 0; u < U; ++u) {
    s1[u] = make_float4(0, 0, 0, 0); s2[u] = make_float4(0, 0, 0, 0);
    mean[u] = *reinterpret_cast<const float4*>(stats + c + 4 * u);
    istd[u] = *reinterpret_cast<const float4*>(stats + C + c + 4 * u);
  }
  for (long r = bv < nbv ? (long)bv * RL1 + vl : rows; r < rows; r += (long)nbv * RL1) {
    const long i0 = r * C4 + (c >> 2);
    float4 xv[U], dv[U];
    ldv<T, U>(x, i0 / U, xv);
    ldv<T, U>(dy, i0 / U, dv);
#pragma unroll
    for (int u = 0; u < U; ++u) {
      const float4 g = bn_masked_grad<T>(dv[u], xv[u], yact, i0 + u, stats, C, c + 4 * u, mask_mode);
      s1[u].x += g.x; s1[u].y += g.y; s1[u].z += g.z; s1[u].w += g.w;
      s2[u].x = fmaf(g.x, (xv[u].x - mean[u].x) * istd[u].x, s2[u].x); s2[u].y = fmaf(g.y, (xv[u].y - mean[u].y) * istd[u].y, s2[u].y);
      s2[u].z = fmaf(g.z, (xv[u].z - mean[u].z) * istd[u].z, s2[u].z); s2[u].w = fmaf(g.w, (xv[u].w - mean[u].w) * istd[u].w, s2[u].w);
    }
  }
#pragma unroll
  for (int u = 0; u < U; ++u) {
    float* d = sm + ((long)rl * CC + cq * 4 * U + 4 * u) * 2;
    d[0] = s1[u].x; d[1] = s2[u].x; d[2] = s1[u].y; d[3] = s2[u].y; d[4] = s1[u].z; d[5] = s2[u].z; d[6] = s1[u].w; d[7] = s2[u].w;
  }
  __syncthreads();
  for (int j = threadIdx.x; j < 2 * CC; j += NP_THREADS) {
#pragma unroll
    for (int h = 0; h < U; ++h) {
      if (blockIdx.x * U + h >= nbv) break;
      float s = 0.f;
      for (int q = h * RL1; q < (h + 1) * RL1; ++q) s += sm[(long)q * 2 * CC + j];
      partial[(long)(blockIdx.x * U + h) * 2 * C + 2 * c0 + j] = s;
    }
  }
}

struct CoefSeg { int T1; long pstride; double count1; int S0, S1; };
__global__ void bn_bwd_coef_kernel(const float* __restrict__ part, int T, int C, double count, const float* __restrict__ gamma,
                                   const float* __restrict__ stats, float* __restrict__ coef, float* __restrict__ dgamma,
                                   float* __restrict__ dbeta, int accumulate, double* __restrict__ scratch, unsigned* __restrict__ tickets,
                                   CoefSeg cs) {
  __shared__ double sm[CS_LANES][CS_COLS];
  __shared__ double tot[CS_COLS];
  __shared__ int s_last;
  int S = 0;
  const bool seg = gridDim.z > 1;
  if (seg) {
    if (blockIdx.z) { part += cs.pstride; T = cs.T1; count = cs.count1; stats += 5 * C; coef += 5 * C; scratch += (long)(CS_MAX_SLICES + 2) * 2 * C; tickets += LMKD_TICKET_WORDS / 2; S = cs.S1; }
    else S = cs.S0;
  }
  if (!colsum_ticket(part, T, 2 * C, scratch, tickets, sm, tot, &s_last, nullptr, S)) return;
  const int c = blockIdx.x * (CS_COLS / 2) + threadIdx.x;
  if (threadIdx.y != 0 || threadIdx.x >= CS_COLS / 2 || c >= C) return;
  const double sg = tot[2 * threadIdx.x], sgx = tot[2 * threadIdx.x + 1];
  const float g = gamma ? gamma[c] : 1.f;
  const float invstd = stats[C + c];
  coef[c] = g * invstd;
  coef[C + c] = (float)(sg / count);
  coef[2 * C + c] = (float)(sgx / count);
  if (seg) {
    coef[3 * C + c] = (float)sgx;
    coef[4 * C + c] = (float)sg;
    return;
  }
  if (dgamma) dgamma[c] = accumulate ? dgamma[c] + (float)sgx : (float)sgx;
  if (dbeta) dbeta[c] = accumulate ? dbeta[c] + (float)sg : (float)sg;
}

struct ParamGradSeg { float* dgamma; float* dbeta; int accumulate; };
__device__ __forceinline__ void bn_param_grads_seg(const float* __restrict__ coef, int C, const ParamGradSeg& pg) {
  if (blockIdx.x != 0 || !pg.dgamma) return;
  for (int c = threadIdx.x; c < C; c += blockDim.x) {
    const float gx = coef[3 * C + c] + coef[5 * C + 3 * C + c], g = coef[4 * C + c] + coef[5 * C + 4 * C + c];
    pg.dgamma[c] = pg.accumulate ? pg.dgamma[c] + gx : gx;
    if (pg.dbeta) pg.dbeta[c] = pg.accumulate ? pg.dbeta[c] + g : g;
  }
}

template <typename T>
__global__ void bn_bwd_apply_kernel(const T* __restrict__ dy, const T* __restrict__ x, const T* __restrict__ yact,
                                    const float* __restrict__ stats, const float* __restrict__ coef, T* __restrict__ dx,
                                    T* __restrict__ g_out, long n4, int C, int mask_mode, long n4_0, ParamGradSeg pg,
                                    unsigned* __restrict__ amax, const unsigned* __restrict__ aref) {
  constexpr int U = ActU<T>::U;
  const int C4 = C >> 2;
  const long nu = n4 / U;
  if (n4_0 < n4) bn_param_grads_seg(coef, C, pg);
  AmaxStat am = {0.f, 0.f, 0u}, am1 = {0.f, 0.f, 0u};
  const AmaxRef rf0 = amax_ref(aref ? amax_read(aref, 0) : 0u), rf1 = amax_ref(aref ? amax_read(aref, 1) : 0u);
  for (long iu = (long)blockIdx.x * blockDim.x + threadIdx.x; iu < nu; iu += (long)gridDim.x * blockDim.x) {
    float4 xv[U], dv[U], o[U], gq[U];
    ldv<T, U>(x, iu, xv);
    ldv<T, U>(dy, iu, dv);
    const int so = iu * U >= n4_0 ? 5 * C : 0;
    const float* st = stats + so;
    const float* cf = coef + so;
#pragma unroll
    for (int u = 0; u < U; ++u) {
      const long i = iu * U + u;
      const int c = (int)(i % C4) * 4;
      const float4 g = bn_masked_grad<T>(dv[u], xv[u], yact, i, st, C, c, mask_mode);
      const float4 mean = *reinterpret_cast<const float4*>(st + c);
      const float4 istd = *reinterpret_cast<const float4*>(st + C + c);
      const float4 A = *reinterpret_cast<const float4*>(cf + c);
      const float4 mg = *reinterpret_cast<const float4*>(cf + C + c);
      const float4 mgx = *reinterpret_cast<const float4*>(cf + 2 * C + c);
      o[u].x = A.x * (g.x - mg.x - (xv[u].x - mean.x) * istd.x * mgx.x);
      o[u].y = A.y * (g.y - mg.y - (xv[u].y - mean.y) * istd.y * mgx.y);
      o[u].z = A.z * (g.z - mg.z - (xv[u].z - mean.z) * istd.z * mgx.z);
      o[u].w = A.w * (g.w - mg.w - (xv[u].w - mean.w) * istd.w * mgx.w);
      gq[u] = g;
      if (so) amax_stat4(am1, o[u], rf1); else amax_stat4(am, o[u], rf0);
    }
    stv<T, U>(dx, iu, o);
    if (g_out) stv<T, U>(g_out, iu, gq);
  }
  if (amax) {
    amax_commit_stat(amax, am, aref != nullptr);
    if (n4_0 < n4) amax_commit_stat(amax + LMKD_AMAX_SEG_WORDS, am1, aref != nullptr);
  }
}

extern "C" long lmkd_bn_bwd_workspace(int C) { return (long)(2048 * 2 * C) * sizeof(float) + (long)(66 * 2 * C) * sizeof(double) + 64; }

static int bn_bwd_stats_impl(const float* dy, const float* x, const float* yact, const float* stats, const float* gamma, float* dgamma,
                             float* dbeta, float* coef, void* workspace, unsigned* tickets, long rows, long count, int C, int mask_mode,
                             int accumulate_param_grads, hipStream_t s, const char* who, long rows0 = 0, long count0 = 0) {
  LMKD_REQUIRE(dy && x && stats && coef && workspace && tickets, "%s: null pointer", who);
  const bool seg = rows0 > 0 && rows0 < rows;
  LMKD_REQUIRE(!seg || cdiv(2 * C, CS_COLS) <= LMKD_TICKET_WORDS / 2, "%s: C=%d exceeds the ticket buffer", who, C);
  const int CC = C > 1024 ? 1024 : C;
  const int U = g_lmkd_act_bf16 ? 2 : 1;
  LMKD_REQUIRE(C % (4 * U) == 0 && C % CC == 0 && 256 % (CC / 4) == 0, "%s: unsupported channel count %d", who, C);
  LMKD_REQUIRE((mask_mode != 1 && mask_mode != 3) || yact, "%s: mask_mode 1 / 3 needs the activation output / its bit mask", who);
  LMKD_REQUIRE(mask_mode != 3 || C % 32 == 0, "%s: bit masks need C %% 32 == 0", who);
  LMKD_REQUIRE(cdiv(2 * C, CS_COLS) <= LMKD_TICKET_WORDS, "%s: C=%d exceeds the ticket buffer", who, C);
  const int RL1 = NP_THREADS / (CC / 4), RL = RL1 * U;
  auto blocks = [&](long r) {
    int nb = cdiv(r, (long)RL1 * 8);
    if (nb > 256 * g_ew_wg_per_cu * 2) nb = 256 * g_ew_wg_per_cu * 2;
    if (nb > 2048) nb = 2048;
    return nb < 1 ? 1 : nb;
  };
  const int nb = blocks(seg ? rows0 : rows), nb1 = seg ? blocks(rows - rows0) : 0;
  const int nbx = std::max(nb, nb1);
  float* partial = (float*)workspace;
  double* dscr = (double*)((char*)workspace + (((long)(seg ? 2 : 1) * 2048 * 2 * C * sizeof(float) + 63) / 64) * 64);
  BnSeg bs;
  bs.rows0 = seg ? rows0 : rows; bs.nb1 = nb1;
  const int gz = seg ? 2 : 1;
  if (g_lmkd_act_bf16)
    hipLaunchKernelGGL(bn_bwd_reduce_kernel<lmkd_bf16_t>, dim3(cdiv(nbx, 2), C / CC, gz), dim3(NP_THREADS), (size_t)RL * CC * 2 * sizeof(float), s,
                       (const lmkd_bf16_t*)dy, (const lmkd_bf16_t*)x, (const lmkd_bf16_t*)yact, stats, partial, rows, C, CC, mask_mode, nb, bs);
  else
    hipLaunchKernelGGL(bn_bwd_reduce_kernel<float>, dim3(nbx, C / CC, gz), dim3(NP_THREADS), (size_t)RL * CC * 2 * sizeof(float), s, dy, x, yact,
                       stats, partial, rows, C, CC, mask_mode, nb, bs);
  LMKD_CHECK_LAUNCH("bn_bwd_reduce_kernel");
  CoefSeg cs;
  cs.T1 = nb1; cs.pstride = (long)2048 * 2 * C; cs.count1 = (double)(count - count0); cs.S0 = cs_slices(nb); cs.S1 = seg ? cs_slices(nb1) : 0;
  hipLaunchKernelGGL(bn_bwd_coef_kernel, dim3(cdiv(2 * C, CS_COLS), std::max(cs.S0, cs.S1), gz), dim3(CS_COLS, CS_LANES), 0, s, (const float*)partial, nb, C,
                     (double)(seg ? count0 : count), gamma, stats, coef, dgamma, dbeta, accumulate_param_grads, dscr, tickets, cs);
  LMKD_CHECK_LAUNCH("bn_bwd_coef_kernel");
  return LMKD_OK;
}

extern "C" int lmkd_bn_backward_seg(const float* dy, const float* x, const float* yact, const float* stats, const float* gamma, float* dx,
                                    float* g_out, float* dgamma, float* dbeta, float* coef, void* workspace, unsigned* tickets, long rows,
                                    long rows0, int C, int mask_mode, int accumulate_param_grads, void* stream, const lmkd_amax_desc* amd);
extern "C" int lmkd_bn_backward(const float* dy, const float* x, const float* yact, const float* stats, const float* gamma,
                                float* dx, float* g_out, float* dgamma, float* dbeta, float* coef, void* workspace, unsigned* tickets,
                                long rows, int C, int mask_mode, int accumulate_param_grads, void* stream) {
  return lmkd_bn_backward_seg(dy, x, yact, stats, gamma, dx, g_out, dgamma, dbeta, coef, workspace, tickets, rows, rows, C, mask_mode,
                              accumulate_param_grads, stream, nullptr);
}
extern "C" int lmkd_bn_backward_seg(const float* dy, const float* x, const float* yact, const float* stats, const float* gamma, float* dx,
                                    float* g_out, float* dgamma, float* dbeta, float* coef, void* workspace, unsigned* tickets, long rows,
                                    long rows0, int C, int mask_mode, int accumulate_param_grads, void* stream, const lmkd_amax_desc* amd) {
  unsigned* amax = amd_out(amd);
  const unsigned* aref = amd_ref(amd);
  LMKD_REQUIRE(dx, "lmkd_bn_backward: null pointer");
  hipStream_t s = (hipStream_t)stream;
  if (rows0 <= 0 || rows0 >= rows) rows0 = rows;
  const int rc = bn_bwd_stats_impl(dy, x, yact, stats, gamma, dgamma, dbeta, coef, workspace, tickets, rows, rows, C, mask_mode,
                                   accumulate_param_grads, s, "lmkd_bn_backward", rows0, rows0);
  if (rc) return rc;
  const long n4 = rows * C / 4, n4_0 = rows0 * C / 4;
  ParamGradSeg pg;
  pg.dgamma = dgamma; pg.dbeta = dbeta; pg.accumulate = accumulate_param_grads;
  if (g_lmkd_act_bf16)
    hipLaunchKernelGGL(bn_bwd_apply_kernel<lmkd_bf16_t>, dim3(ew_grid(n4)), dim3(NP_THREADS), 0, s, (const lmkd_bf16_t*)dy, (const lmkd_bf16_t*)x,
                       (const lmkd_bf16_t*)yact, stats, (const float*)coef, (lmkd_bf16_t*)dx, (lmkd_bf16_t*)g_out, n4, C, mask_mode, n4_0, pg, amax, aref);
  else
    hipLaunchKernelGGL(bn_bwd_apply_kernel<float>, dim3(ew_grid(n4)), dim3(NP_THREADS), 0, s, dy, x, yact, stats, (const float*)coef, dx, g_out,
                       n4, C, mask_mode, n4_0, pg, amax, aref);
  LMKD_CHECK_LAUNCH("bn_bwd_apply_kernel");
  return LMKD_OK;
}

extern "C" int lmkd_bn_backward_part_seg(const float* part, int T, int T0, const float* dy, const float* x, const float* stats, const float* gamma,
                                         float* dx, float* dgamma, float* dbeta, float* coef, void* workspace, unsigned* tickets, long rows,
                                         long rows0, int C, int accumulate_param_grads, void* stream, const lmkd_amax_desc* amd);
extern "C" int lmkd_bn_backward_part(const float* part, int T, const float* dy, const float* x, const float* stats, const float* gamma,
                                     float* dx, float* dgamma, float* dbeta, float* coef, void* workspace, unsigned* tickets, long rows, int C,
                                     int accumulate_param_grads, void* stream) {
  return lmkd_bn_backward_part_seg(part, T, T, dy, x, stats, gamma, dx, dgamma, dbeta, coef, workspace, tickets, rows, rows, C,
                                   accumulate_param_grads, stream, nullptr);
}
extern "C" int lmkd_bn_backward_part_seg(const float* part, int T, int T0, const float* dy, const float* x, const float* stats, const float* gamma,
                                         float* dx, float* dgamma, float* dbeta, float* coef, void* workspace, unsigned* tickets, long rows,
                                         long rows0, int C, int accumulate_param_grads, void* stream, const lmkd_amax_desc* amd) {
  unsigned* amax = amd_out(amd);
  const unsigned* aref = amd_ref(amd);
  LMKD_REQUIRE(part && T > 0 && dy && x && stats && dx && coef && workspace && tickets, "lmkd_bn_backward_part: null pointer");
  LMKD_REQUIRE(!g_lmkd_act_bf16 && C % 4 == 0, "lmkd_bn_backward_part: fp32 tensors, C %% 4 == 0");
  const bool seg = T0 > 0 && T0 < T && rows0 > 0 && rows0 < rows;
  LMKD_REQUIRE(seg || (T0 == T && rows0 == rows), "lmkd_bn_backward_part_seg: T0 / rows0 must both name a split or both the whole");
  LMKD_REQUIRE(cdiv(2 * C, CS_COLS) <= LMKD_TICKET_WORDS / (seg ? 2 : 1), "lmkd_bn_backward_part: C=%d exceeds the ticket buffer", C);
  hipStream_t s = (hipStream_t)stream;
  double* dscr = (double*)((char*)workspace + (((long)2048 * 2 * C * sizeof(float) + 63) / 64) * 64);
  CoefSeg cs;
  cs.T1 = T - T0; cs.pstride = (long)T0 * 2 * C; cs.count1 = (double)(rows - rows0); cs.S0 = cs_slices(T0); cs.S1 = seg ? cs_slices(T - T0) : 0;
  hipLaunchKernelGGL(bn_bwd_coef_kernel, dim3(cdiv(2 * C, CS_COLS), std::max(cs.S0, cs.S1), seg ? 2 : 1), dim3(CS_COLS, CS_LANES), 0, s, part, T0, C,
                     (double)rows0, gamma, stats, coef, dgamma, dbeta, accumulate_param_grads, dscr, tickets, cs);
  LMKD_CHECK_LAUNCH("bn_bwd_coef_kernel");
  const long n4 = rows * C / 4;
  ParamGradSeg pg;
  pg.dgamma = dgamma; pg.dbeta = dbeta; pg.accumulate = accumulate_param_grads;
  hipLaunchKernelGGL(bn_bwd_apply_kernel<float>, dim3(ew_grid(n4)), dim3(NP_THREADS), 0, s, dy, x, (const float*)nullptr, stats, (const float*)coef,
                     dx, (float*)nullptr, n4, C, 2, rows0 * C / 4, pg, amax, aref);
  LMKD_CHECK_LAUNCH("bn_bwd_apply_kernel");
  return LMKD_OK;
}

extern "C" int lmkd_bn_backward_stats(const float* dy, const float* cmax, const float* stats, const float* gamma, float* dgamma, float* dbeta,
                                      float* coef, void* workspace, unsigned* tickets, long pooled_rows, long count, int C,
                                      int accumulate_param_grads, void* stream) {
  LMKD_REQUIRE(pooled_rows > 0 && count >= pooled_rows, "lmkd_bn_backward_stats: bad row counts");
  return bn_bwd_stats_impl(dy, cmax, nullptr, stats, gamma, dgamma, dbeta, coef, workspace, tickets, pooled_rows, count, C, 2,
                           accumulate_param_grads, (hipStream_t)stream, "lmkd_bn_backward_stats");
}
extern "C" int lmkd_bn_backward_stats_seg(const float* dy, const float* cmax, const float* stats, const float* gamma, float* coef, void* workspace,
                                          unsigned* tickets, long pooled_rows, long pooled_rows0, long count, long count0, int C, void* stream) {
  LMKD_REQUIRE(pooled_rows0 > 0 && pooled_rows0 < pooled_rows && count0 >= pooled_rows0 && count - count0 >= pooled_rows - pooled_rows0,
               "lmkd_bn_backward_stats_seg: bad row counts");
  return bn_bwd_stats_impl(dy, cmax, nullptr, stats, gamma, nullptr, nullptr, coef, workspace, tickets, pooled_rows, count, C, 2, 0,
                           (hipStream_t)stream, "lmkd_bn_backward_stats_seg", pooled_rows0, count0);
}

template <typename T>
__global__ void relu_bwd_kernel(const T* __restrict__ dy, const T* __restrict__ y, T* __restrict__ g, long n4) {
  for (long i = (long)blockIdx.x * blockDim.x + threadIdx.x; i < n4; i += (long)gridDim.x * blockDim.x) {
    const float4 d = ld4<T>(dy, i), v = ld4<T>(y, i);
    st4<T>(g, i, make_float4(v.x > 0.f ? d.x : 0.f, v.y > 0.f ? d.y : 0.f, v.z > 0.f ? d.z : 0.f, v.w > 0.f ? d.w : 0.f));
  }
}
extern "C" int lmkd_relu_backward(const float* dy, const float* y, float* g, long n, void* stream) {
  LMKD_REQUIRE(dy && y && g && n > 0 && n % 4 == 0, "lmkd_relu_backward: bad arguments");
  if (g_lmkd_act_bf16)
    hipLaunchKernelGGL(relu_bwd_kernel<lmkd_bf16_t>, dim3(ew_grid(n / 4)), dim3(NP_THREADS), 0, (hipStream_t)stream, (const lmkd_bf16_t*)dy,
                       (const lmkd_bf16_t*)y, (lmkd_bf16_t*)g, n / 4);
  else
    hipLaunchKernelGGL(relu_bwd_kernel<float>, dim3(ew_grid(n / 4)), dim3(NP_THREADS), 0, (hipStream_t)stream, dy, y, g, n / 4);
  LMKD_CHECK_LAUNCH("relu_bwd_kernel");
  return LMKD_OK;
}

template <typename T>
__global__ void bn_relu_maxpool_kernel(const T* __restrict__ x, const float* __restrict__ stats, T* __restrict__ y,
                                       uchar4* __restrict__ idx, T* __restrict__ cmax, int N, int H, int W, int C, int OH, int OW, int N0,
                                       unsigned* __restrict__ amax, const unsigned* __restrict__ aref) {
  constexpr int U = ActU<T>::U;
  const int CU = C / (4 * U);
  const long total = (long)N * OH * OW * CU;
  AmaxStat amx = {0.f, 0.f, 0u}, amx1 = {0.f, 0.f, 0u};
  const AmaxRef rf0 = amax_ref(aref ? amax_read(aref, 0) : 0u), rf1 = amax_ref(aref ? amax_read(aref, 1) : 0u);
  for (long i = (long)blockIdx.x * blockDim.x + threadIdx.x; i < total; i += (long)gridDim.x * blockDim.x) {
    const int cq = (int)(i % CU);
    long r = i / CU;
    const int ow = (int)(r % OW); r /= OW;
    const int oh = (int)(r % OH);
    const int n = (int)(r / OH);
    float4 sc[U], sh[U], m[U], cm[U];
    uchar4 am[U];
#pragma unroll
    for (int u = 0; u < U; ++u) {
      const float* st = stats + (n >= N0 ? 5 * C : 0);
      sc[u] = *reinterpret_cast<const float4*>(st + 2 * C + (cq * U + u) * 4);
      sh[u] = *reinterpret_cast<const float4*>(st + 3 * C + (cq * U + u) * 4);
      m[u] = make_float4(-INFINITY, -INFINITY, -INFINITY, -INFINITY);
      cm[u] = make_float4(0.f, 0.f, 0.f, 0.f);
      am[u] = make_uchar4(255, 255, 255, 255);
    }
#pragma unroll
    for (int kh = 0; kh < 3; ++kh) {
      const int h = oh * 2 - 1 + kh;
      if ((unsigned)h >= (unsigned)H) continue;
#pragma unroll
      for (int kw = 0; kw < 3; ++kw) {
        const int w = ow * 2 - 1 + kw;
        if ((unsigned)w >= (unsigned)W) continue;
        float4 rr[U];
        ldv<T, U>(x, ((long)(n * H + h) * W + w) * CU + cq, rr);
        const unsigned char t = (unsigned char)(kh * 3 + kw);
#pragma unroll
        for (int u = 0; u < U; ++u) {
          const float4 r4 = rr[u];
          float4 v;
          v.x = fmaxf(fmaf(r4.x, sc[u].x, sh[u].x), 0.f); v.y = fmaxf(fmaf(r4.y, sc[u].y, sh[u].y), 0.f);
          v.z = fmaxf(fmaf(r4.z, sc[u].z, sh[u].z), 0.f); v.w = fmaxf(fmaf(r4.w, sc[u].w, sh[u].w), 0.f);
          if (v.x > m[u].x || am[u].x == 255) { m[u].x = v.x; am[u].x = t; cm[u].x = r4.x; }
          if (v.y > m[u].y || am[u].y == 255) { m[u].y = v.y; am[u].y = t; cm[u].y = r4.y; }
          if (v.z > m[u].z || am[u].z == 255) { m[u].z = v.z; am[u].z = t; cm[u].z = r4.z; }
          if (v.w > m[u].w || am[u].w == 255) { m[u].w = v.w; am[u].w = t; cm[u].w = r4.w; }
        }
      }
    }
    stv<T, U>(y, i, m);
#pragma unroll
    for (int u = 0; u < U; ++u) {
      idx[i * U + u] = am[u];
      if (n >= N0) amax_stat4(amx1, m[u], rf1); else amax_stat4(amx, m[u], rf0);
    }
    if (cmax) stv<T, U>(cmax, i, cm);
  }
  if (amax) {
    amax_commit_stat(amax, amx, aref != nullptr);
    if (N0 < N) amax_commit_stat(amax + LMKD_AMAX_SEG_WORDS, amx1, aref != nullptr);
  }
}

extern "C" int lmkd_bn_relu_maxpool_fwd_seg(const float* x, const float* stats, float* y, unsigned char* idx, float* cmax, int N, int N0, int H,
                                            int W, int C, void* stream, const lmkd_amax_desc* amd);
extern "C" int lmkd_bn_relu_maxpool_fwd(const float* x, const float* stats, float* y, unsigned char* idx, float* cmax, int N, int H, int W,
                                        int C, void* stream) {
  return lmkd_bn_relu_maxpool_fwd_seg(x, stats, y, idx, cmax, N, N, H, W, C, stream, nullptr);
}
extern "C" int lmkd_bn_relu_maxpool_fwd_seg(const float* x, const float* stats, float* y, unsigned char* idx, float* cmax, int N, int N0, int H,
                                            int W, int C, void* stream, const lmkd_amax_desc* amd) {
  unsigned* amax = amd_out(amd);
  const unsigned* aref = amd_ref(amd);
  LMKD_REQUIRE(x && stats && y && idx && C % (g_lmkd_act_bf16 ? 8 : 4) == 0, "lmkd_bn_relu_maxpool_fwd: bad arguments");
  if (N0 <= 0 || N0 > N) N0 = N;
  const int OH = (H + 2 - 3) / 2 + 1, OW = (W + 2 - 3) / 2 + 1;
  const long total = (long)N * OH * OW * C / (g_lmkd_act_bf16 ? 8 : 4);
  if (g_lmkd_act_bf16)
    hipLaunchKernelGGL(bn_relu_maxpool_kernel<lmkd_bf16_t>, dim3(ew_grid(total)), dim3(NP_THREADS), 0, (hipStream_t)stream, (const lmkd_bf16_t*)x,
                       stats, (lmkd_bf16_t*)y, (uchar4*)idx, (lmkd_bf16_t*)cmax, N, H, W, C, OH, OW, N0, amax, aref);
  else
    hipLaunchKernelGGL(bn_relu_maxpool_kernel<float>, dim3(ew_grid(total)), dim3(NP_THREADS), 0, (hipStream_t)stream, x, stats, y, (uchar4*)idx,
                       cmax, N, H, W, C, OH, OW, N0, amax, aref);
  LMKD_CHECK_LAUNCH("bn_relu_maxpool_kernel");
  return LMKD_OK;
}

template <typename T>
__global__ void maxpool_bwd_kernel(const T* __restrict__ dy, const uchar4* __restrict__ idx, T* __restrict__ g, int N, int H,
                                   int W, int C, int OH, int OW) {
  const int C4 = C >> 2;
  const long total = (long)N * H * W * C4;
  for (long i = (long)blockIdx.x * blockDim.x + threadIdx.x; i < total; i += (long)gridDim.x * blockDim.x) {
    const int cq = (int)(i % C4);
    long r = i / C4;
    const int w = (int)(r % W); r /= W;
    const int h = (int)(r % H);
    const int n = (int)(r / H);
    float4 acc = make_float4(0.f, 0.f, 0.f, 0.f);
    const int oh_lo = h >> 1, oh_hi = (h + 1) >> 1;
    const int ow_lo = w >> 1, ow_hi = (w + 1) >> 1;
    for (int oh = oh_lo; oh <= oh_hi; ++oh) {
      if (oh >= OH) continue;
      const int kh = h - (2 * oh - 1);
      for (int ow = ow_lo; ow <= ow_hi; ++ow) {
        if (ow >= OW) continue;
        const int kw = w - (2 * ow - 1);
        const unsigned char t = (unsigned char)(kh * 3 + kw);
        const long o = ((long)(n * OH + oh) * OW + ow) * C4 + cq;
        const uchar4 am = idx[o];
        const float4 d = ld4<T>(dy, o);
        if (am.x == t) acc.x += d.x;
        if (am.y == t) acc.y += d.y;
        if (am.z == t) acc.z += d.z;
        if (am.w == t) acc.w += d.w;
      }
    }
    st4<T>(g, i, acc);
  }
}

template <typename T>
__global__ void stem_unpool_bn_bwd_kernel(const T* __restrict__ dy, const uchar4* __restrict__ idx, const T* __restrict__ c,
                                          const float* __restrict__ stats, const float* __restrict__ coef, T* __restrict__ dc, int N,
                                          int H, int W, int C, int OH, int OW, int N0, ParamGradSeg pg, unsigned* __restrict__ amax,
                                          const unsigned* __restrict__ aref) {
  const int C4 = C >> 2;
  const int HB = (H + 1) >> 1, WB = (W + 1) >> 1;
  const long total = (long)N * HB * WB * C4;
  AmaxStat amx = {0.f, 0.f, 0u}, amx1 = {0.f, 0.f, 0u};
  const AmaxRef rf0 = amax_ref(aref ? amax_read(aref, 0) : 0u), rf1 = amax_ref(aref ? amax_read(aref, 1) : 0u);
  if (N0 < N) bn_param_grads_seg(coef, C, pg);
  for (long i = (long)blockIdx.x * blockDim.x + threadIdx.x; i < total; i += (long)gridDim.x * blockDim.x) {
    const int cq = (int)(i % C4);
    long r = i / C4;
    const int b = (int)(r % WB); r /= WB;
    const int a = (int)(r % HB);
    const int n = (int)(r / HB);
    const int ch = cq * 4 + (n >= N0 ? 5 * C : 0);
    const float4 sc = *reinterpret_cast<const float4*>(stats + 2 * C + ch);
    const float4 sh = *reinterpret_cast<const float4*>(stats + 3 * C + ch);
    const float4 mean = *reinterpret_cast<const float4*>(stats + ch);
    const float4 istd = *reinterpret_cast<const float4*>(stats + C + ch);
    const float4 A = *reinterpret_cast<const float4*>(coef + ch);
    const float4 mg = *reinterpret_cast<const float4*>(coef + C + ch);
    const float4 mgx = *reinterpret_cast<const float4*>(coef + 2 * C + ch);
    float4 d[2][2];
    uchar4 am[2][2];
#pragma unroll
    for (int wi = 0; wi < 2; ++wi)
#pragma unroll
      for (int wj = 0; wj < 2; ++wj) {
        const int oh = a + wi, ow = b + wj;
        if (oh < OH && ow < OW) {
          const long o = ((long)(n * OH + oh) * OW + ow) * C4 + cq;
          d[wi][wj] = ld4<T>(dy, o);
          am[wi][wj] = idx[o];
        } else {
          d[wi][wj] = make_float4(0.f, 0.f, 0.f, 0.f);
          am[wi][wj] = make_uchar4(254, 254, 254, 254);
        }
      }
#pragma unroll
    for (int pi = 0; pi < 2; ++pi) {
      const int h = 2 * a + pi;
      if (h >= H) continue;
#pragma unroll
      for (int pj = 0; pj < 2; ++pj) {
        const int w = 2 * b + pj;
        if (w >= W) continue;
        float4 g = make_float4(0.f, 0.f, 0.f, 0.f);
#pragma unroll
        for (int wi = 0; wi <= pi; ++wi) {
          const int kh = wi == 0 ? pi + 1 : 0;
#pragma unroll
          for (int wj = 0; wj <= pj; ++wj) {
            const int kw = wj == 0 ? pj + 1 : 0;
            const unsigned char t = (unsigned char)(kh * 3 + kw);
            if (am[wi][wj].x == t) g.x += d[wi][wj].x;
            if (am[wi][wj].y == t) g.y += d[wi][wj].y;
            if (am[wi][wj].z == t) g.z += d[wi][wj].z;
            if (am[wi][wj].w == t) g.w += d[wi][wj].w;
          }
        }
        const long p = ((long)(n * H + h) * W + w) * C4 + cq;
        const float4 xv = ld4<T>(c, p);
        g.x = fmaf(xv.x, sc.x, sh.x) > 0.f ? g.x : 0.f; g.y = fmaf(xv.y, sc.y, sh.y) > 0.f ? g.y : 0.f;
        g.z = fmaf(xv.z, sc.z, sh.z) > 0.f ? g.z : 0.f; g.w = fmaf(xv.w, sc.w, sh.w) > 0.f ? g.w : 0.f;
        float4 o;
        o.x = A.x * (g.x - mg.x - (xv.x - mean.x) * istd.x * mgx.x);
        o.y = A.y * (g.y - mg.y - (xv.y - mean.y) * istd.y * mgx.y);
        o.z = A.z * (g.z - mg.z - (xv.z - mean.z) * istd.z * mgx.z);
        o.w = A.w * (g.w - mg.w - (xv.w - mean.w) * istd.w * mgx.w);
        st4<T>(dc, p, o);
        if (n >= N0) amax_stat4(amx1, o, rf1); else amax_stat4(amx, o, rf0);
      }
    }
  }
  if (amax) {
    amax_commit_stat(amax, amx, aref != nullptr);
    if (N0 < N) amax_commit_stat(amax + LMKD_AMAX_SEG_WORDS, amx1, aref != nullptr);
  }
}

extern "C" int lmkd_stem_unpool_bn_bwd_seg(const float* dy, const unsigned char* idx, const float* c, const float* stats, const float* coef,
                                           float* dc, float* dgamma, float* dbeta, int accumulate_param_grads, int N, int N0, int H, int W, int C,
                                           void* stream, const lmkd_amax_desc* amd);
extern "C" int lmkd_stem_unpool_bn_bwd(const float* dy, const unsigned char* idx, const float* c, const float* stats, const float* coef,
                                       float* dc, int N, int H, int W, int C, void* stream, const lmkd_amax_desc* amd) {
  return lmkd_stem_unpool_bn_bwd_seg(dy, idx, c, stats, coef, dc, nullptr, nullptr, 0, N, N, H, W, C, stream, amd);
}
extern "C" int lmkd_stem_unpool_bn_bwd_seg(const float* dy, const unsigned char* idx, const float* c, const float* stats, const float* coef,
                                           float* dc, float* dgamma, float* dbeta, int accumulate_param_grads, int N, int N0, int H, int W, int C,
                                           void* stream, const lmkd_amax_desc* amd) {
  unsigned* amax = amd_out(amd);
  const unsigned* aref = amd_ref(amd);
  LMKD_REQUIRE(dy && idx && c && stats && coef && dc && C % 4 == 0 && N > 0 && H > 0 && W > 0, "lmkd_stem_unpool_bn_bwd: bad arguments");
  if (N0 <= 0 || N0 > N) N0 = N;
  ParamGradSeg pg;
  pg.dgamma = dgamma; pg.dbeta = dbeta; pg.accumulate = accumulate_param_grads;
  const int OH = (H + 2 - 3) / 2 + 1, OW = (W + 2 - 3) / 2 + 1;
  const long total = (long)N * ((H + 1) / 2) * ((W + 1) / 2) * C / 4;
  if (g_lmkd_act_bf16)
    hipLaunchKernelGGL(stem_unpool_bn_bwd_kernel<lmkd_bf16_t>, dim3(ew_grid(total)), dim3(NP_THREADS), 0, (hipStream_t)stream,
                       (const lmkd_bf16_t*)dy, (const uchar4*)idx, (const lmkd_bf16_t*)c, stats, coef, (lmkd_bf16_t*)dc, N, H, W, C, OH, OW, N0, pg, amax, aref);
  else
    hipLaunchKernelGGL(stem_unpool_bn_bwd_kernel<float>, dim3(ew_grid(total)), dim3(NP_THREADS), 0, (hipStream_t)stream, dy, (const uchar4*)idx, c,
                       stats, coef, dc, N, H, W, C, OH, OW, N0, pg, amax, aref);
  LMKD_CHECK_LAUNCH("stem_unpool_bn_bwd_kernel");
  return LMKD_OK;
}

extern "C" int lmkd_maxpool_bwd(const float* dy, const unsigned char* idx, float* g, int N, int H, int W, int C, void* stream) {
  LMKD_REQUIRE(dy && idx && g && C % 4 == 0, "lmkd_maxpool_bwd: bad arguments");
  const int OH = (H + 2 - 3) / 2 + 1, OW = (W + 2 - 3) / 2 + 1;
  const long total = (long)N * H * W * C / 4;
  if (g_lmkd_act_bf16)
    hipLaunchKernelGGL(maxpool_bwd_kernel<lmkd_bf16_t>, dim3(ew_grid(total)), dim3(NP_THREADS), 0, (hipStream_t)stream, (const lmkd_bf16_t*)dy,
                       (const uchar4*)idx, (lmkd_bf16_t*)g, N, H, W, C, OH, OW);
  else
    hipLaunchKernelGGL(maxpool_bwd_kernel<float>, dim3(ew_grid(total)), dim3(NP_THREADS), 0, (hipStream_t)stream, dy, (const uchar4*)idx, g, N, H,
                       W, C, OH, OW);
  LMKD_CHECK_LAUNCH("maxpool_bwd_kernel");
  return LMKD_OK;
}

template <typename T>
__global__ void adaptive_maxpool_mean_kernel(const T* __restrict__ x, float* __restrict__ y, int F, int H, int W, int C) {
  const long total = (long)F * C;
  for (long i = (long)blockIdx.x * blockDim.x + threadIdx.x; i < total; i += (long)gridDim.x * blockDim.x) {
    const int c = (int)(i % C);
    const int f = (int)(i / C);
    const T* b = x + (long)f * H * W * C + c;
    float s = 0.f;
    for (int ph = 0; ph < 4; ++ph) {
      const int h0 = (ph * H) / 4, h1 = ((ph + 1) * H + 3) / 4;
      for (int pw = 0; pw < 4; ++pw) {
        const int w0 = (pw * W) / 4, w1 = ((pw + 1) * W + 3) / 4;
        float m = -INFINITY;
        for (int h = h0; h < h1; ++h)
          for (int w = w0; w < w1; ++w) m = fmaxf(m, ld1<T>(b, (long)(h * W + w) * C));
        s += m;
      }
    }
    y[i] = s * (1.f / 16.f);
// ... 87 lines not shown
```

Baseline: 51.06.

## Template BN elementwise kernels on mode, use 32-bit indexing and incremental channel walk

The BN apply, backward-reduce and backward-apply kernels now take the residual/mask mode (and g_out presence) as template parameters. This removes runtime branches and lets dead paths compile away. Per-element 64-bit modulo channel math is replaced by a wave-uniform incremental ModWalk and 32-bit byte offsets, and the split-segment check is hoisted into a two-segment outer loop. The wgrad split-reduce kernel switches to 32-bit offsets with a new size guard. Compiler barriers and ds_swizzle shuffles aim to cut VALU and scalar overhead, at the cost of more kernel instantiations and tighter index-range limits.

Measured after the change: 51.54 (median of 6 runs). About the same (+0.9%).

```diff
diff --git a/lite-mkd_amd/csrc/conv.hip b/lite-mkd_amd/csrc/conv.hip
--- a/lite-mkd_amd/csrc/conv.hip
+++ b/lite-mkd_amd/csrc/conv.hip
@@ -456,26 +456,29 @@
   }
 }
 
-__global__ void wgrad_reduce_kernel(const float* __restrict__ slab, float* __restrict__ dw, int splits, int Co, int Cin,
-                                    int Cs, int KH, int KW, int KWp, int Kp, int accumulate) {
-  const long total = (long)Co * KH * KW * Cin;
-  const long zs = (long)Co * Kp;
-  for (long idx = (long)blockIdx.x * blockDim.x + threadIdx.x; idx < total; idx += (long)gridDim.x * blockDim.x) {
-    const int ci = idx % Cin;
-    long r = idx / Cin;
-    const int kw = r % KW; r /= KW;
-    const int kh = r % KH;
-    const int co = r / KH;
-    const float* p = slab + (long)co * Kp + (long)(kh * KWp + kw) * Cs + ci;
+__global__ void __launch_bounds__(256) wgrad_reduce_kernel(const float* __restrict__ slab, float* __restrict__ dw, int splits, int Co, int Cin,
+                                                           int Cs, int KH, int KW, int KWp, int Kp, int accumulate) {
+  const unsigned total = (unsigned)Co * KH * KW * Cin;
+  const long zs = (long)Co * Kp * 4;
+  const char* sb = reinterpret_cast<const char*>(slab);
+  for (unsigned idx = blockIdx.x * 256u + threadIdx.x; idx < total; idx += gridDim.x * 256u) {
+    const unsigned ci = idx % (unsigned)Cin;
+    unsigned r = idx / (unsigned)Cin;
+    const unsigned kw = r % (unsigned)KW; r /= (unsigned)KW;
+    const unsigned kh = r % (unsigned)KH;
+    const unsigned co = r / (unsigned)KH;
+    unsigned off = (co * Kp + (kh * KWp + kw) * Cs + ci) * 4u;
+    auto at = [&](int z) { return *reinterpret_cast<const float*>(sb + z * zs + off); };
     float s0 = 0.f, s1 = 0.f, s2 = 0.f, s3 = 0.f;
     int z = 0;
     for (; z + 8 <= splits; z += 8) {
-      const float a0 = p[(z + 0) * zs], a1 = p[(z + 1) * zs], a2 = p[(z + 2) * zs], a3 = p[(z + 3) * zs];
-      const float a4 = p[(z + 4) * zs], a5 = p[(z + 5) * zs], a6 = p[(z + 6) * zs], a7 = p[(z + 7) * zs];
+      asm volatile("" : "+v"(off));
+      const float a0 = at(z + 0), a1 = at(z + 1), a2 = at(z + 2), a3 = at(z + 3);
+      const float a4 = at(z + 4), a5 = at(z + 5), a6 = at(z + 6), a7 = at(z + 7);
       s0 += a0; s1 += a1; s2 += a2; s3 += a3; s0 += a4; s1 += a5; s2 += a6; s3 += a7;
     }
-    for (; z < splits; ++z) s0 += p[z * zs];
-    float* o = dw + (((long)co * Cin + ci) * KH + kh) * KW + kw;
+    for (; z < splits; ++z) s0 += at(z);
+    float* o = dw + ((co * Cin + ci) * KH + kh) * KW + kw;
     const float v = (s0 + s1) + (s2 + s3);
     *o = accumulate ? *o + v : v;
   }
@@ -509,12 +512,14 @@
     }
   }
 }
-static void launch_wgrad_reduce(const float* slab, float* dw, int splits, int Co, int Cin, int Cs, int KH, int KW, int KWp, int Kp,
-                                int accumulate, hipStream_t s) {
+static int launch_wgrad_reduce(const float* slab, float* dw, int splits, int Co, int Cin, int Cs, int KH, int KW, int KWp, int Kp,
+                               int accumulate, hipStream_t s) {
   const long total = (long)Co * KH * KW * Cin;
+  LMKD_REQUIRE(total < 2147483647L && (long)Co * Kp < (1L << 30), "wgrad_reduce: %ld weights / slabs of %ld floats exceed its 32-bit indices", total, (long)Co * Kp);
   int rg = cdiv(total, 256);
   if (rg > 4096) rg = 4096;
   hipLaunchKernelGGL(wgrad_reduce_kernel, dim3(rg), dim3(256), 0, s, slab, dw, splits, Co, Cin, Cs, KH, KW, KWp, Kp, accumulate);
+  return LMKD_OK;
 }
 
 #include "wgrad_x3.h"
@@ -1649,7 +1654,7 @@
       hipLaunchKernelGGL(wgrad_reduce_stem_kernel, dim3(Cout), dim3(256, 4), 0, s, (const float*)workspace, dw_oihw, p.splits, Cout, Cin, Cs, KH, KW,
                          KWp, Kp, accumulate);
     } else {
-      launch_wgrad_reduce((const float*)workspace, dw_oihw, p.splits, Cout, Cin, Cs, KH, KW, KWp, Kp, accumulate, s);
+      if (const int rc = launch_wgrad_reduce((const float*)workspace, dw_oihw, p.splits, Cout, Cin, Cs, KH, KW, KWp, Kp, accumulate, s)) return rc;
     }
     LMKD_CHECK_LAUNCH("wgrad_reduce_kernel");
     return LMKD_OK;
@@ -1670,7 +1675,7 @@
     if (p.cob == 4) launch_wgrad_win<4>(w, p, big, s);
     else launch_wgrad_win<2>(w, p, big, s);
     LMKD_CHECK_LAUNCH("conv_wgrad_win_kernel");
-    launch_wgrad_reduce((const float*)workspace, dw_oihw, p.splits, Cout, Cin, Cs, KH, KW, KWp, Kp, accumulate, s);
+    if (const int rc = launch_wgrad_reduce((const float*)workspace, dw_oihw, p.splits, Cout, Cin, Cs, KH, KW, KWp, Kp, accumulate, s)) return rc;
     LMKD_CHECK_LAUNCH("wgrad_reduce_kernel");
     return LMKD_OK;
   }
@@ -1703,7 +1708,7 @@
     else launch_wgrad_tile<TileCfg<128, 128, 2, 4>, false, 512>(a, p, s);
     LMKD_CHECK_LAUNCH("conv_wgrad_kernel");
   }
-  launch_wgrad_reduce((const float*)workspace, dw_oihw, p.splits, Cout, Cin, Cs, KH, KW, KWp, Kp, accumulate, s);
+  if (const int rc = launch_wgrad_reduce((const float*)workspace, dw_oihw, p.splits, Cout, Cin, Cs, KH, KW, KWp, Kp, accumulate, s)) return rc;
   LMKD_CHECK_LAUNCH("wgrad_reduce_kernel");
   return LMKD_OK;
 }
diff --git a/lite-mkd_amd/csrc/norm_pool.hip b/lite-mkd_amd/csrc/norm_pool.hip
--- a/lite-mkd_amd/csrc/norm_pool.hip
+++ b/lite-mkd_amd/csrc/norm_pool.hip
@@ -10,6 +10,29 @@
   g_ew_wg_per_cu = n;
   return LMKD_OK;
 }
+
+__device__ __forceinline__ unsigned np_after(unsigned c, const float4& w) {
+  asm volatile("" : "+v"(c) : "v"(w.x), "v"(w.y), "v"(w.z), "v"(w.w));
+  return c;
+}
+__device__ __forceinline__ float4 ldtab(const float* __restrict__ tab, unsigned c) {
+  return *reinterpret_cast<const float4*>(reinterpret_cast<const char*>(tab) + c * 4u);
+}
+__device__ __forceinline__ AmaxRef amax_ref_uniform(const unsigned* __restrict__ aref, int seg) {
+  AmaxRef r = amax_ref(aref ? amax_read(aref, seg) : 0u);
+  r.thr = __uint_as_float(__builtin_amdgcn_readfirstlane(__float_as_uint(r.thr)));
+  r.inv_thr = __uint_as_float(__builtin_amdgcn_readfirstlane(__float_as_uint(r.inv_thr)));
+  return r;
+}
+template <int K> __device__ __forceinline__ unsigned lane_xor(unsigned v) { return (unsigned)__builtin_amdgcn_ds_swizzle((int)v, (K << 10) | 0x1f); }
+struct ModWalk {
+  unsigned q, step, n;
+  __device__ __forceinline__ ModWalk(int n_) : n((unsigned)n_) {
+    q = (blockIdx.x * (unsigned)NP_THREADS + threadIdx.x) % n;
+    step = (unsigned)__builtin_amdgcn_readfirstlane((int)((gridDim.x * (unsigned)NP_THREADS) % n));
+  }
+  __device__ __forceinline__ void next() { q += step; q = q >= n ? q - n : q; }
+};
 static inline int ew_grid(long n_items) {
   long g = (n_items + NP_THREADS - 1) / NP_THREADS;
   if (g > 256 * g_ew_wg_per_cu) g = 256 * g_ew_wg_per_cu;
@@ -481,53 +504,57 @@
   return LMKD_OK;
 }
 
-template <typename T>
-__global__ void bn_apply_kernel(const T* __restrict__ x, const float* __restrict__ stats, const T* __restrict__ res,
-                                const float* __restrict__ rstats, T* __restrict__ y, long n4, int C, int relu, int res_mode,
+template <typename T, int RES_MODE>
+__global__ void __launch_bounds__(NP_THREADS) bn_apply_kernel(const T* __restrict__ x, const float* __restrict__ stats, const T* __restrict__ res,
+                                const float* __restrict__ rstats, T* __restrict__ y, long n4, int C, int relu,
                                 unsigned* __restrict__ mask_bits, long n4_0, unsigned* __restrict__ amax, const unsigned* __restrict__ aref) {
   constexpr int U = ActU<T>::U;
-  const int C4 = C >> 2;
-  const long nu = n4 / U;
-  AmaxStat am = {0.f, 0.f, 0u}, am1 = {0.f, 0.f, 0u};
-  const AmaxRef rf0 = amax_ref(aref ? amax_read(aref, 0) : 0u), rf1 = amax_ref(aref ? amax_read(aref, 1) : 0u);
-  for (long iu = (long)blockIdx.x * blockDim.x + threadIdx.x; iu < nu; iu += (long)gridDim.x * blockDim.x) {
-    float4 v[U], r[U];
-    ldv<T, U>(x, iu, v);
-    if (res_mode) ldv<T, U>(res, iu, r);
-    unsigned nibs = 0;
-    const int so = iu * U >= n4_0 ? 5 * C : 0;
-#pragma unroll
-    for (int u = 0; u < U; ++u) {
-      const long i = iu * U + u;
-      const int c = (int)(i % C4) * 4 + so;
-      const float4 sc = *reinterpret_cast<const float4*>(stats + 2 * C + c);
-      const float4 sh = *reinterpret_cast<const float4*>(stats + 3 * C + c);
-      float4& w = v[u];
-      w.x = fmaf(w.x, sc.x, sh.x); w.y = fmaf(w.y, sc.y, sh.y); w.z = fmaf(w.z, sc.z, sh.z); w.w = fmaf(w.w, sc.w, sh.w);
-      if (res_mode == 1) {
-        w.x += r[u].x; w.y += r[u].y; w.z += r[u].z; w.w += r[u].w;
-      } else if (res_mode == 2) {
-        const float4 rs = *reinterpret_cast<const float4*>(rstats + 2 * C + c);
-        const float4 rh = *reinterpret_cast<const float4*>(rstats + 3 * C + c);
-        w.x += fmaf(r[u].x, rs.x, rh.x); w.y += fmaf(r[u].y, rs.y, rh.y); w.z += fmaf(r[u].z, rs.z, rh.z); w.w += fmaf(r[u].w, rs.w, rh.w);
+  const AmaxRef rf0 = amax_ref_uniform(aref, 0), rf1 = amax_ref_uniform(aref, 1);
+  ModWalk cw(C / (4 * U));
+  long iu = (long)blockIdx.x * NP_THREADS + threadIdx.x;
+#pragma unroll 1
+  for (int seg = 0; seg < 2; ++seg) {
+    const long nu = (seg ? n4 : n4_0) / U;
+    const unsigned so = seg ? 5u * C : 0u;
+    const AmaxRef rf = seg ? rf1 : rf0;
+    AmaxStat am = {0.f, 0.f, 0u};
+    for (; iu < nu; iu += (long)gridDim.x * NP_THREADS, cw.next()) {
+      float4 v[U], r[U];
+      ldv<T, U>(x, iu, v);
+      if (RES_MODE) ldv<T, U>(res, iu, r);
+      unsigned nibs = 0;
+#pragma unroll
+      for (int u = 0; u < U; ++u) {
+        const unsigned c = (cw.q * U + u) * 4 + so;
+        float4& w = v[u];
+        {
+          const float4 sc = ldtab(stats + 2 * C, c);
+          const float4 sh = ldtab(stats + 3 * C, c);
+          w.x = fmaf(w.x, sc.x, sh.x); w.y = fmaf(w.y, sc.y, sh.y); w.z = fmaf(w.z, sc.z, sh.z); w.w = fmaf(w.w, sc.w, sh.w);
+        }
+        if (RES_MODE == 1) {
+          w.x += r[u].x; w.y += r[u].y; w.z += r[u].z; w.w += r[u].w;
+        } else if (RES_MODE == 2) {
+          const unsigned c2 = np_after(c, w);
+          const float4 rs = ldtab(rstats + 2 * C, c2);
+          const float4 rh = ldtab(rstats + 3 * C, c2);
+          w.x += fmaf(r[u].x, rs.x, rh.x); w.y += fmaf(r[u].y, rs.y, rh.y); w.z += fmaf(r[u].z, rs.z, rh.z); w.w += fmaf(r[u].w, rs.w, rh.w);
+        }
+        w.x = relu ? fmaxf(w.x, 0.f) : w.x; w.y = relu ? fmaxf(w.y, 0.f) : w.y; w.z = relu ? fmaxf(w.z, 0.f) : w.z; w.w = relu ? fmaxf(w.w, 0.f) : w.w;
+        nibs |= ((w.x > 0.f ? 1u : 0u) | (w.y > 0.f ? 2u : 0u) | (w.z > 0.f ? 4u : 0u) | (w.w > 0.f ? 8u : 0u)) << (4 * u);
+        amax_stat4(am, w, rf);
       }
-      if (relu) { w.x = fmaxf(w.x, 0.f); w.y = fmaxf(w.y, 0.f); w.z = fmaxf(w.z, 0.f); w.w = fmaxf(w.w, 0.f); }
-      nibs |= ((w.x > 0.f ? 1u : 0u) | (w.y > 0.f ? 2u : 0u) | (w.z > 0.f ? 4u : 0u) | (w.w > 0.f ? 8u : 0u)) << (4 * u);
-      if (so) amax_stat4(am1, w, rf1); else amax_stat4(am, w, rf0);
-    }
-    stv<T, U>(y, iu, v);
-    if (mask_bits) {
-      constexpr int LPW = 8 / U;
-      unsigned wbits = nibs << (4 * U * (threadIdx.x & (LPW - 1)));
-      wbits |= __shfl_xor(wbits, 1, 64);
-      wbits |= __shfl_xor(wbits, 2, 64);
-      if (LPW == 8) wbits |= __shfl_xor(wbits, 4, 64);
-      if ((threadIdx.x & (LPW - 1)) == 0) mask_bits[iu / LPW] = wbits;
-    }
-  }
-  if (amax) {
-    amax_commit_stat(amax, am, aref != nullptr);
-    if (n4_0 < n4) amax_commit_stat(amax + LMKD_AMAX_SEG_WORDS, am1, aref != nullptr);
+      stv<T, U>(y, iu, v);
+      if (mask_bits) {
+        constexpr int LPW = 8 / U;
+        unsigned wbits = nibs << (4 * U * (threadIdx.x & (LPW - 1)));
+        wbits |= lane_xor<1>(wbits);
+        wbits |= lane_xor<2>(wbits);
+        if (LPW == 8) wbits |= lane_xor<4>(wbits);
+        if ((threadIdx.x & (LPW - 1)) == 0) mask_bits[iu / LPW] = wbits;
+      }
+    }
+    if (amax && (seg == 0 || n4_0 < n4)) amax_commit_stat(amax + seg * LMKD_AMAX_SEG_WORDS, am, aref != nullptr);
   }
 }
 
@@ -548,47 +575,53 @@
   LMKD_REQUIRE(!mask_bits || C % 32 == 0, "lmkd_bn_apply: the ReLU bit mask needs C %% 32 == 0 (C=%d)", C);
   LMKD_REQUIRE(!g_lmkd_act_bf16 || C % 8 == 0, "lmkd_bn_apply: bf16 tensors need C %% 8 == 0 (C=%d)", C);
   const long n4 = rows * C / 4;
-  if (g_lmkd_act_bf16)
-    hipLaunchKernelGGL(bn_apply_kernel<lmkd_bf16_t>, dim3(ew_grid(n4)), dim3(NP_THREADS), 0, (hipStream_t)stream, (const lmkd_bf16_t*)x, stats,
-                       (const lmkd_bf16_t*)res, rstats, (lmkd_bf16_t*)y, n4, C, relu, res_mode, mask_bits, rows0 * C / 4, amax, aref);
-  else
-    hipLaunchKernelGGL(bn_apply_kernel<float>, dim3(ew_grid(n4)), dim3(NP_THREADS), 0, (hipStream_t)stream, x, stats, res, rstats, y, n4, C,
-                       relu, res_mode, mask_bits, rows0 * C / 4, amax, aref);
+#define LMKD_BN_APPLY(T, RM)                                                                                                              \
+  hipLaunchKernelGGL((bn_apply_kernel<T, RM>), dim3(ew_grid(n4)), dim3(NP_THREADS), 0, (hipStream_t)stream, (const T*)x, stats, (const T*)res, \
+                     rstats, (T*)y, n4, C, relu, mask_bits, rows0 * C / 4, amax, aref)
+  LMKD_REQUIRE(res_mode >= 0 && res_mode <= 2, "lmkd_bn_apply: res_mode %d", res_mode);
+  if (g_lmkd_act_bf16) {
+    if (res_mode == 0) LMKD_BN_APPLY(lmkd_bf16_t, 0); else if (res_mode == 1) LMKD_BN_APPLY(lmkd_bf16_t, 1); else LMKD_BN_APPLY(lmkd_bf16_t, 2);
+  } else {
+    if (res_mode == 0) LMKD_BN_APPLY(float, 0); else if (res_mode == 1) LMKD_BN_APPLY(float, 1); else LMKD_BN_APPLY(float, 2);
+  }
+#undef LMKD_BN_APPLY
   LMKD_CHECK_LAUNCH("bn_apply_kernel");
   return LMKD_OK;
 }
 
-template <typename T>
+template <typename T, int MASK_MODE>
 __device__ __forceinline__ float4 bn_masked_grad(const float4 dy, const float4 xv, const T* yact, long i, const float* stats,
-                                                 int C, int c, int mask_mode) {
+                                                 int C, unsigned c) {
   float4 g = dy;
-  if (mask_mode == 3) {
+  if (MASK_MODE == 3) {
     const unsigned nib = (reinterpret_cast<const unsigned*>(yact)[i >> 3] >> (4 * (int)(i & 7))) & 15u;
     g.x = (nib & 1u) ? g.x : 0.f; g.y = (nib & 2u) ? g.y : 0.f; g.z = (nib & 4u) ? g.z : 0.f; g.w = (nib & 8u) ? g.w : 0.f;
-  } else if (mask_mode == 1) {
+  } else if (MASK_MODE == 1) {
     const float4 yv = ld4<T>(yact, i);
     g.x = yv.x > 0.f ? g.x : 0.f; g.y = yv.y > 0.f ? g.y : 0.f; g.z = yv.z > 0.f ? g.z : 0.f; g.w = yv.w > 0.f ? g.w : 0.f;
-  } else if (mask_mode == 2) {
-    const float4 sc = *reinterpret_cast<const float4*>(stats + 2 * C + c);
-    const float4 sh = *reinterpret_cast<const float4*>(stats + 3 * C + c);
-    g.x = fmaf(xv.x, sc.x, sh.x) > 0.f ? g.x : 0.f; g.y = fmaf(xv.y, sc.y, sh.y) > 0.f ? g.y : 0.f;
-    g.z = fmaf(xv.z, sc.z, sh.z) > 0.f ? g.z : 0.f; g.w = fmaf(xv.w, sc.w, sh.w) > 0.f ? g.w : 0.f;
+  } else if (MASK_MODE == 2) {
+    const float4 sc = ldtab(stats + 2 * C, c);
+    const float4 sh = ldtab(stats + 3 * C, c);
+    unsigned nib = (fmaf(xv.x, sc.x, sh.x) > 0.f ? 1u : 0u) | (fmaf(xv.y, sc.y, sh.y) > 0.f ? 2u : 0u) |
+                   (fmaf(xv.z, sc.z, sh.z) > 0.f ? 4u : 0u) | (fmaf(xv.w, sc.w, sh.w) > 0.f ? 8u : 0u);
+    asm volatile("" : "+v"(nib));
+    g.x = (nib & 1u) ? g.x : 0.f; g.y = (nib & 2u) ? g.y : 0.f; g.z = (nib & 4u) ? g.z : 0.f; g.w = (nib & 8u) ? g.w : 0.f;
   }
   return g;
 }
 
 struct BnSeg { long rows0; int nb1; };
-template <typename T>
-__global__ void bn_bwd_reduce_kernel(const T* __restrict__ dy, const T* __restrict__ x, const T* __restrict__ yact,
+template <typename T, int MASK_MODE>
+__global__ void __launch_bounds__(NP_THREADS) bn_bwd_reduce_kernel(const T* __restrict__ dy, const T* __restrict__ x, const T* __restrict__ yact,
                                      const float* __restrict__ stats, float* __restrict__ partial, long rows, int C, int CC,
-                                     int mask_mode, int nbv, BnSeg sg) {
+                                     int nbv, BnSeg sg) {
   extern __shared__ float sm[];
   constexpr int U = ActU<T>::U;
   if (gridDim.z > 1) {
     if (blockIdx.z) {
       const long eo = sg.rows0 * C;
       dy += eo; x += eo;
-      if (yact) yact = mask_mode == 3 ? reinterpret_cast<const T*>(reinterpret_cast<const unsigned*>(yact) + eo / 32) : yact + eo;
+      if (yact) yact = MASK_MODE == 3 ? reinterpret_cast<const T*>(reinterpret_cast<const unsigned*>(yact) + eo / 32) : yact + eo;
       stats += 5 * C; partial += (long)2048 * 2 * C; rows -= sg.rows0; nbv = sg.nb1;
     } else {
       rows = sg.rows0;
@@ -600,29 +633,31 @@
   const int bv = blockIdx.x * U + rl / RL1, vl = rl % RL1;
   const int c0 = blockIdx.y * CC;
   const int c = c0 + cq * 4 * U;
-  float4 s1[U], s2[U], mean[U], istd[U];
-#pragma unroll
-  for (int u = 0; u < U; ++u) {
-    s1[u] = make_float4(0, 0, 0, 0); s2[u] = make_float4(0, 0, 0, 0);
-    mean[u] = *reinterpret_cast<const float4*>(stats + c + 4 * u);
-    istd[u] = *reinterpret_cast<const float4*>(stats + C + c + 4 * u);
-  }
-  for (long r = bv < nbv ? (long)bv * RL1 + vl : rows; r < rows; r += (long)nbv * RL1) {
-    const long i0 = r * C4 + (c >> 2);
+  float4 s1[U], s2[U];
+#pragma unroll
+  for (int u = 0; u < U; ++u) { s1[u] = make_float4(0, 0, 0, 0); s2[u] = make_float4(0, 0, 0, 0); }
+  const long iend = rows * C4, istep = (long)nbv * RL1 * C4;
+  for (long i0 = bv < nbv ? ((long)bv * RL1 + vl) * C4 + (c >> 2) : iend; i0 < iend; i0 += istep) {
+    asm volatile("" : "+v"(i0));
     float4 xv[U], dv[U];
     ldv<T, U>(x, i0 / U, xv);
     ldv<T, U>(dy, i0 / U, dv);
 #pragma unroll
     for (int u = 0; u < U; ++u) {
-      const float4 g = bn_masked_grad<T>(dv[u], xv[u], yact, i0 + u, stats, C, c + 4 * u, mask_mode);
+      unsigned cu = (unsigned)c + 4 * u;
+      asm volatile("" : "+v"(cu));
+      const float4 g = bn_masked_grad<T, MASK_MODE>(dv[u], xv[u], yact, i0 + u, stats, C, cu);
       s1[u].x += g.x; s1[u].y += g.y; s1[u].z += g.z; s1[u].w += g.w;
-      s2[u].x = fmaf(g.x, (xv[u].x - mean[u].x) * istd[u].x, s2[u].x); s2[u].y = fmaf(g.y, (xv[u].y - mean[u].y) * istd[u].y, s2[u].y);
-      s2[u].z = fmaf(g.z, (xv[u].z - mean[u].z) * istd[u].z, s2[u].z); s2[u].w = fmaf(g.w, (xv[u].w - mean[u].w) * istd[u].w, s2[u].w);
+      const unsigned c1 = np_after(cu, g);
+      const float4 mean = ldtab(stats, c1);
+      const float4 istd = ldtab(stats + C, c1);
+      s2[u].x = fmaf(g.x, (xv[u].x - mean.x) * istd.x, s2[u].x); s2[u].y = fmaf(g.y, (xv[u].y - mean.y) * istd.y, s2[u].y);
+      s2[u].z = fmaf(g.z, (xv[u].z - mean.z) * istd.z, s2[u].z); s2[u].w = fmaf(g.w, (xv[u].w - mean.w) * istd.w, s2[u].w);
     }
   }
 #pragma unroll
   for (int u = 0; u < U; ++u) {
-    float* d = sm + ((long)rl * CC + cq * 4 * U + 4 * u) * 2;
+    float* d = sm + (rl * CC + cq * 4 * U + 4 * u) * 2;
     d[0] = s1[u].x; d[1] = s2[u].x; d[2] = s1[u].y; d[3] = s2[u].y; d[4] = s1[u].z; d[5] = s2[u].z; d[6] = s1[u].w; d[7] = s2[u].w;
   }
   __syncthreads();
@@ -679,48 +714,71 @@
   }
 }
 
-template <typename T>
-__global__ void bn_bwd_apply_kernel(const T* __restrict__ dy, const T* __restrict__ x, const T* __restrict__ yact,
+template <typename T, int MASK_MODE, bool GOUT>
+__global__ void __launch_bounds__(NP_THREADS) bn_bwd_apply_kernel(const T* __restrict__ dy, const T* __restrict__ x, const T* __restrict__ yact,
                                     const float* __restrict__ stats, const float* __restrict__ coef, T* __restrict__ dx,
-                                    T* __restrict__ g_out, long n4, int C, int mask_mode, long n4_0, ParamGradSeg pg,
+                                    T* __restrict__ g_out, long n4, int C, long n4_0, ParamGradSeg pg,
                                     unsigned* __restrict__ amax, const unsigned* __restrict__ aref) {
   constexpr int U = ActU<T>::U;
-  const int C4 = C >> 2;
-  const long nu = n4 / U;
   if (n4_0 < n4) bn_param_grads_seg(coef, C, pg);
-  AmaxStat am = {0.f, 0.f, 0u}, am1 = {0.f, 0.f, 0u};
-  const AmaxRef rf0 = amax_ref(aref ? amax_read(aref, 0) : 0u), rf1 = amax_ref(aref ? amax_read(aref, 1) : 0u);
-  for (long iu = (long)blockIdx.x * blockDim.x + threadIdx.x; iu < nu; iu += (long)gridDim.x * blockDim.x) {
-    float4 xv[U], dv[U], o[U], gq[U];
-    ldv<T, U>(x, iu, xv);
-    ldv<T, U>(dy, iu, dv);
-    const int so = iu * U >= n4_0 ? 5 * C : 0;
-    const float* st = stats + so;
-    const float* cf = coef + so;
-#pragma unroll
-    for (int u = 0; u < U; ++u) {
-      const long i = iu * U + u;
-      const int c = (int)(i % C4) * 4;
-      const float4 g = bn_masked_grad<T>(dv[u], xv[u], yact, i, st, C, c, mask_mode);
-      const float4 mean = *reinterpret_cast<const float4*>(st + c);
-      const float4 istd = *reinterpret_cast<const float4*>(st + C + c);
-      const float4 A = *reinterpret_cast<const float4*>(cf + c);
-      const float4 mg = *reinterpret_cast<const float4*>(cf + C + c);
-      const float4 mgx = *reinterpret_cast<const float4*>(cf + 2 * C + c);
-      o[u].x = A.x * (g.x - mg.x - (xv[u].x - mean.x) * istd.x * mgx.x);
-      o[u].y = A.y * (g.y - mg.y - (xv[u].y - mean.y) * istd.y * mgx.y);
-      o[u].z = A.z * (g.z - mg.z - (xv[u].z - mean.z) * istd.z * mgx.z);
-      o[u].w = A.w * (g.w - mg.w - (xv[u].w - mean.w) * istd.w * mgx.w);
-      gq[u] = g;
-      if (so) amax_stat4(am1, o[u], rf1); else amax_stat4(am, o[u], rf0);
-    }
-    stv<T, U>(dx, iu, o);
-    if (g_out) stv<T, U>(g_out, iu, gq);
-  }
-  if (amax) {
-    amax_commit_stat(amax, am, aref != nullptr);
-    if (n4_0 < n4) amax_commit_stat(amax + LMKD_AMAX_SEG_WORDS, am1, aref != nullptr);
-  }
+  const AmaxRef rf0 = amax_ref_uniform(aref, 0), rf1 = amax_ref_uniform(aref, 1);
+  ModWalk cw(C / (4 * U));
+  long iu = (long)blockIdx.x * NP_THREADS + threadIdx.x;
+#pragma unroll 1
+  for (int seg = 0; seg < 2; ++seg) {
+    const long nu = (seg ? n4 : n4_0) / U;
+    const unsigned so = seg ? 5u * C : 0u;
+    const AmaxRef rf = seg ? rf1 : rf0;
+    AmaxStat am = {0.f, 0.f, 0u};
+    for (; iu < nu; iu += (long)gridDim.x * NP_THREADS, cw.next()) {
+      float4 xv[U], dv[U];
+      ldv<T, U>(x, iu, xv);
+      ldv<T, U>(dy, iu, dv);
+#pragma unroll
+      for (int u = 0; u < U; ++u) {
+        const unsigned c = (cw.q * U + u) * 4 + so;
+        dv[u] = bn_masked_grad<T, MASK_MODE>(dv[u], xv[u], yact, iu * U + u, stats, C, c);
+        const unsigned c1 = np_after(c, dv[u]);
+        const float4 mean = ldtab(stats, c1);
+        const float4 istd = ldtab(stats + C, c1);
+        xv[u].x = (xv[u].x - mean.x) * istd.x; xv[u].y = (xv[u].y - mean.y) * istd.y;
+        xv[u].z = (xv[u].z - mean.z) * istd.z; xv[u].w = (xv[u].w - mean.w) * istd.w;
+      }
+      if (GOUT) stv<T, U>(g_out, iu, dv);
+#pragma unroll
+      for (int u = 0; u < U; ++u) {
+        const unsigned c2 = np_after((cw.q * U + u) * 4 + so, xv[u]);
+        float4& o = dv[u];
+        {
+          const float4 mgx = ldtab(coef + 2 * C, c2);
+          const float4 mg = ldtab(coef + C, c2);
+          o.x = o.x - mg.x - xv[u].x * mgx.x; o.y = o.y - mg.y - xv[u].y * mgx.y;
+          o.z = o.z - mg.z - xv[u].z * mgx.z; o.w = o.w - mg.w - xv[u].w * mgx.w;
+        }
+        const float4 A = ldtab(coef, np_after(c2, o));
+        o.x = A.x * o.x; o.y = A.y * o.y; o.z = A.z * o.z; o.w = A.w * o.w;
+        amax_stat4(am, o, rf);
+      }
+      stv<T, U>(dx, iu, dv);
+    }
+    if (amax && (seg == 0 || n4_0 < n4)) amax_commit_stat(amax + seg * LMKD_AMAX_SEG_WORDS, am, aref != nullptr);
+  }
+}
+
+template <typename T>
+static void bn_bwd_apply_launch(hipStream_t s, const void* dy, const void* x, const void* yact, const float* stats, const float* coef, void* dx,
+                                void* g_out, long n4, int C, int mask_mode, long n4_0, ParamGradSeg pg, unsigned* amax, const unsigned* aref) {
+#define LMKD_BWD_APPLY(MM, GO)                                                                                                         \
+  hipLaunchKernelGGL((bn_bwd_apply_kernel<T, MM, GO>), dim3(ew_grid(n4)), dim3(NP_THREADS), 0, s, (const T*)dy, (const T*)x, (const T*)yact, \
+                     stats, coef, (T*)dx, (T*)g_out, n4, C, n4_0, pg, amax, aref)
+  if (g_out) {
+    if (mask_mode == 0) LMKD_BWD_APPLY(0, true); else if (mask_mode == 1) LMKD_BWD_APPLY(1, true);
+    else if (mask_mode == 2) LMKD_BWD_APPLY(2, true); else LMKD_BWD_APPLY(3, true);
+  } else {
+    if (mask_mode == 0) LMKD_BWD_APPLY(0, false); else if (mask_mode == 1) LMKD_BWD_APPLY(1, false);
+    else if (mask_mode == 2) LMKD_BWD_APPLY(2, false); else LMKD_BWD_APPLY(3, false);
+  }
+#undef LMKD_BWD_APPLY
 }
 
 extern "C" long lmkd_bn_bwd_workspace(int C) { return (long)(2048 * 2 * C) * sizeof(float) + (long)(66 * 2 * C) * sizeof(double) + 64; }
@@ -751,12 +809,18 @@
   BnSeg bs;
   bs.rows0 = seg ? rows0 : rows; bs.nb1 = nb1;
   const int gz = seg ? 2 : 1;
-  if (g_lmkd_act_bf16)
-    hipLaunchKernelGGL(bn_bwd_reduce_kernel<lmkd_bf16_t>, dim3(cdiv(nbx, 2), C / CC, gz), dim3(NP_THREADS), (size_t)RL * CC * 2 * sizeof(float), s,
-                       (const lmkd_bf16_t*)dy, (const lmkd_bf16_t*)x, (const lmkd_bf16_t*)yact, stats, partial, rows, C, CC, mask_mode, nb, bs);
-  else
-    hipLaunchKernelGGL(bn_bwd_reduce_kernel<float>, dim3(nbx, C / CC, gz), dim3(NP_THREADS), (size_t)RL * CC * 2 * sizeof(float), s, dy, x, yact,
-                       stats, partial, rows, C, CC, mask_mode, nb, bs);
+  LMKD_REQUIRE(mask_mode >= 0 && mask_mode <= 3, "%s: mask_mode %d", who, mask_mode);
+#define LMKD_BWD_REDUCE(T, MM, GX)                                                                                                        \
+  hipLaunchKernelGGL((bn_bwd_reduce_kernel<T, MM>), dim3(GX, C / CC, gz), dim3(NP_THREADS), (size_t)RL * CC * 2 * sizeof(float), s, (const T*)dy, \
+                     (const T*)x, (const T*)yact, stats, partial, rows, C, CC, nb, bs)
+  if (g_lmkd_act_bf16) {
+    if (mask_mode == 0) LMKD_BWD_REDUCE(lmkd_bf16_t, 0, cdiv(nbx, 2)); else if (mask_mode == 1) LMKD_BWD_REDUCE(lmkd_bf16_t, 1, cdiv(nbx, 2));
+    else if (mask_mode == 2) LMKD_BWD_REDUCE(lmkd_bf16_t, 2, cdiv(nbx, 2)); else LMKD_BWD_REDUCE(lmkd_bf16_t, 3, cdiv(nbx, 2));
+  } else {
+    if (mask_mode == 0) LMKD_BWD_REDUCE(float, 0, nbx); else if (mask_mode == 1) LMKD_BWD_REDUCE(float, 1, nbx);
+    else if (mask_mode == 2) LMKD_BWD_REDUCE(float, 2, nbx); else LMKD_BWD_REDUCE(float, 3, nbx);
+  }
+#undef LMKD_BWD_REDUCE
   LMKD_CHECK_LAUNCH("bn_bwd_reduce_kernel");
   CoefSeg cs;
   cs.T1 = nb1; cs.pstride = (long)2048 * 2 * C; cs.count1 = (double)(count - count0); cs.S0 = cs_slices(nb); cs.S1 = seg ? cs_slices(nb1) : 0;
@@ -789,12 +853,8 @@
   const long n4 = rows * C / 4, n4_0 = rows0 * C / 4;
   ParamGradSeg pg;
   pg.dgamma = dgamma; pg.dbeta = dbeta; pg.accumulate = accumulate_param_grads;
-  if (g_lmkd_act_bf16)
-    hipLaunchKernelGGL(bn_bwd_apply_kernel<lmkd_bf16_t>, dim3(ew_grid(n4)), dim3(NP_THREADS), 0, s, (const lmkd_bf16_t*)dy, (const lmkd_bf16_t*)x,
-                       (const lmkd_bf16_t*)yact, stats, (const float*)coef, (lmkd_bf16_t*)dx, (lmkd_bf16_t*)g_out, n4, C, mask_mode, n4_0, pg, amax, aref);
-  else
-    hipLaunchKernelGGL(bn_bwd_apply_kernel<float>, dim3(ew_grid(n4)), dim3(NP_THREADS), 0, s, dy, x, yact, stats, (const float*)coef, dx, g_out,
-                       n4, C, mask_mode, n4_0, pg, amax, aref);
+  if (g_lmkd_act_bf16) bn_bwd_apply_launch<lmkd_bf16_t>(s, dy, x, yact, stats, coef, dx, g_out, n4, C, mask_mode, n4_0, pg, amax, aref);
+  else bn_bwd_apply_launch<float>(s, dy, x, yact, stats, coef, dx, g_out, n4, C, mask_mode, n4_0, pg, amax, aref);
   LMKD_CHECK_LAUNCH("bn_bwd_apply_kernel");
   return LMKD_OK;
 }
@@ -828,8 +888,7 @@
   const long n4 = rows * C / 4;
   ParamGradSeg pg;
   pg.dgamma = dgamma; pg.dbeta = dbeta; pg.accumulate = accumulate_param_grads;
-  hipLaunchKernelGGL(bn_bwd_apply_kernel<float>, dim3(ew_grid(n4)), dim3(NP_THREADS), 0, s, dy, x, (const float*)nullptr, stats, (const float*)coef,
-                     dx, (float*)nullptr, n4, C, 2, rows0 * C / 4, pg, amax, aref);
+  bn_bwd_apply_launch<float>(s, dy, x, nullptr, stats, coef, dx, nullptr, n4, C, 2, rows0 * C / 4, pg, amax, aref);
   LMKD_CHECK_LAUNCH("bn_bwd_apply_kernel");
   return LMKD_OK;
 }
```
